# soedinglab/plass

Measured on AMD Instinct MI355X. Metric: read-overlaps/s per assembly iteration, higher is better.
Workload: dtype u8/u64 (integer hash, byte compare; f32 ratios)

## Files before the change

plass_amd/csrc/common.hpp:

```cpp
#pragma once
#include <hip/hip_runtime.h>
#include <cstdint>
#include <cstddef>
#include <cstdio>
#include <atomic>
#include <functional>
#include <memory>
#include <mutex>
#include <string>
#include <vector>
#include "../../include/plasship.h"

namespace plasship {

void setError(const std::string &msg);
hipError_t streamSync(hipStream_t st);
}
struct plasship_seqdb; struct plasship_ctx;
namespace plasship {
int ensureOffLen(plasship_ctx *ctx, const plasship_seqdb *db);
std::string hipErrStr(hipError_t e, const char *what, const char *file, int line);

#define PH_CHECK(call)                                                                   \
    do {                                                                                 \
        hipError_t e_ = (call);                                                          \
        if (e_ != hipSuccess) {                                                          \
            plasship::setError(plasship::hipErrStr(e_, #call, __FILE__, __LINE__));     \
            return PLASSHIP_ERR_DEVICE;                                                  \
        }                                                                                \
    } while (0)
#define PH_COPY_SYNC(st, dst, src, bytes, kind)                                          \
    do {                                                                                 \
        PH_CHECK(hipMemcpyAsync((dst), (src), (bytes), (kind), (st)));                   \
        PH_CHECK(plasship::streamSync(st));                                              \
    } while (0)

int tuneInt(const char *name, int dflt);
bool traceOn();
#define PH_TRACE(st, what)                                                                \
    do {                                                                                 \
        if (plasship::traceOn()) {                                                       \
            hipError_t e_ = plasship::streamSync(st);                                    \
            fprintf(stderr, "[plasship] %s: %s\n", (what), hipGetErrorString(e_));       \
        }                                                                                \
    } while (0)

hipError_t poolMalloc(void **p, size_t n, bool longLived = false);
void poolEnter(hipStream_t stream);
void watchEnter(const plasship_ctx *ctx);
void watchCollective(const char *what);
#define PH_ENTER(ctx)                                                                    \
    do {                                                                                 \
        PH_CHECK(hipSetDevice((ctx)->device));                                           \
        plasship::poolEnter((ctx)->stream);                                              \
        plasship::watchEnter(ctx);                                                       \
    } while (0)
void poolFree(void *p);
void poolTrim();

struct DevBuf {
    void *p = nullptr; size_t bytes = 0;
    DevBuf() {}
    DevBuf(const DevBuf &) = delete; DevBuf &operator=(const DevBuf &) = delete;
    ~DevBuf() { release(); }
    hipError_t alloc(size_t n, bool longLived = false) { release(); bytes = n; if (n == 0) { p = nullptr; return hipSuccess; } return poolMalloc(&p, n, longLived); }
    hipError_t allocLong(size_t n) { return alloc(n, true); }
    void release() { if (p) { poolFree(p); p = nullptr; } bytes = 0; }
    template <typename T> T *as() const { return reinterpret_cast<T *>(p); }
};

struct SeqView {
    const char *data;
    const uint64_t *off;
    const uint32_t *len;
    const uint64_t *offLen;
    uint32_t n;
    int nucl;
};

#ifdef __HIPCC__
__device__ __forceinline__ uint64_t seqOff(const SeqView &s, uint32_t id) { return s.offLen[id] >> 24; }
__device__ __forceinline__ uint32_t seqLen(const SeqView &s, uint32_t id) { return (uint32_t) s.offLen[id] & 0xFFFFFFu; }
#endif

struct __attribute__((aligned(8))) CandHit { uint32_t target; int32_t prefScore; uint32_t diag16; uint32_t query; };

struct AlnRec {
    uint32_t query, target;
    int32_t bitScore, rawScore;
    float seqId;
    int32_t qStart, qEnd, qLen, dbStart, dbEnd, dbLen, alnLen;
    int32_t reversed;
    int32_t accepted;
    int32_t fromText;
    int32_t btKind;
};
constexpr int32_t ALN_SELF_PENDING = 3;

}

struct plasship_ctx {
    int device = 0;
    hipStream_t stream = nullptr;
    hipEvent_t ev[16] = {};
    int numCU = 0;
    std::vector<uint32_t> ambKeys;
    std::vector<uint8_t> ambVals;
    plasship::DevBuf d_ambKeys, d_ambVals;
    plasship::DevBuf d_cmpCache;
    uint32_t ambSlots = 0;
    char *stage[2] = {nullptr, nullptr};
    hipEvent_t stageEv[2] = {nullptr, nullptr};
    size_t stageBytes = 0;
    void *pinnedTable = nullptr;
    bool hasComm = false;
    plasship_comm comm = {};
    int debugFailCollective = -1;
    struct KmCache {
        plasship::DevBuf lines; uint64_t n = 0, gen = 0; bool valid = false, seenEligible = false;
        int k = 0, alph = 0, kps = 0, ignoreMulti = 0, hashShift = 0;
    } kmCache;
    struct KmPosCache {
        plasship::DevBuf pos, slotOff, idHash; uint64_t n = 0, gen = 0; bool valid = false, seen = false, lng = false;
        int k = 0, kps = 0, ignoreMulti = 0, hashShift = 0; float scale = 0;
    } kmPosCache;
    uint64_t kmermatchCalls = 0;
    uint64_t cycKnownGen = 0, cycKnownMaxLen = 0;
};

namespace plasship {
uint64_t newDbGeneration();
struct SeqHeap { DevBuf buf; std::atomic<uint64_t> used{0}; };
}
struct plasship_seqdb {
    int dbtype = 0;
    uint64_t gen = plasship::newDbGeneration(), parentGen = 0, ancestorGen = 0;
    plasship::DevBuf d_changed;
    uint64_t originGen = 0;
    plasship::DevBuf d_origin;
    size_t n = 0;
    uint64_t dataBytes = 0, residues = 0;
    uint32_t maxEntryLen = 0;
    plasship::DevBuf d_data, d_off, d_len, d_key;
    std::shared_ptr<plasship::SeqHeap> heap;
    bool contiguous = true;
    uint64_t buildAppendedBytes = 0, buildCopiedBytes = 0;
    const char *borrowedData = nullptr;
    const char *dataPtr() const { return heap ? heap->buf.as<char>() : borrowedData ? borrowedData : d_data.as<char>(); }
    plasship::DevBuf d_fileRank;
    mutable plasship::DevBuf d_offLen;
    mutable std::mutex offLenMu; mutable hipEvent_t offLenEv = nullptr; mutable hipStream_t offLenStream = nullptr;
    ~plasship_seqdb() { if (offLenEv) (void) hipEventDestroy(offLenEv); }
    bool hostIndexValid = false;
    std::vector<uint32_t> h_key, h_elen;
    std::vector<uint64_t> h_off;
    plasship::SeqView view() const {
        plasship::SeqView v; v.data = dataPtr(); v.off = d_off.as<uint64_t>(); v.len = d_len.as<uint32_t>(); v.offLen = d_offLen.as<uint64_t>();
        v.n = (uint32_t) n; v.nucl = (dbtype == PLASSHIP_DBTYPE_NUCLEOTIDES); return v;
    }
};

struct plasship_cands {
    bool reverseCapable = false;
    size_t nQueries = 0;
    uint64_t nHits = 0;
    uint64_t nNonSelf = 0;
    plasship::DevBuf d_qoff;
    plasship::DevBuf d_hits;
};

struct plasship_alns {
    size_t nQueries = 0;
    uint64_t nLines = 0;
    uint64_t nSlots = 0;
    bool sparse = false;
    mutable bool selfPending = false;
    plasship_rescore_params rsPar = {};
    bool rsSameDB = false; int rsReverseCapable = 0;
    bool nucl = false;
    bool addBacktrace = false;
    uint64_t dbResidues = 0;
    int gappedOpen = 0, gappedExtend = 0;
    plasship::DevBuf d_qoff;
    plasship::DevBuf d_recs;
    const plasship_seqdb *qdb = nullptr, *tdb = nullptr;
};

namespace plasship {
inline const plasship_comm *commOf(const plasship_ctx *ctx) { return ctx->hasComm ? &ctx->comm : nullptr; }
inline uint64_t ownedBegin(uint64_t n, int r, int world) { return ((uint64_t) r * n + (uint64_t) world - 1) / (uint64_t) world; }
int commAllgatherHost(plasship_ctx *ctx, const void *send, void *recv, uint64_t bytesPerRank);
int commAllReduceSumU64(plasship_ctx *ctx, uint64_t *v, size_t n);
int commAllReduceMaxU64(plasship_ctx *ctx, uint64_t *v, size_t n);
int commAllReduceMinU64(plasship_ctx *ctx, uint64_t *v, size_t n);
int commAgreeOk(plasship_ctx *ctx, bool ok, const char *what);
int commFinish(plasship_ctx *ctx, int rc);
int commAlltoallvRecords(plasship_ctx *ctx, const void *dSend, const uint64_t *sendCount, size_t recordBytes, DevBuf &recv,
                         uint64_t *recvTotal, uint64_t slackRecords, uint64_t *allTotal = nullptr);
int commAllgathervBytes(plasship_ctx *ctx, const void *dSend, uint64_t sendBytes, DevBuf &recv, std::vector<uint64_t> &recvBytes);
int commAllgathervBytesKnown(plasship_ctx *ctx, const void *dSend, uint64_t sendBytes, DevBuf &recv, const std::vector<uint64_t> &recvBytes);
int packedCopyOf(plasship_ctx *ctx, const plasship_seqdb *db, std::unique_ptr<plasship_seqdb> &out);
int buildOutputDB(plasship_ctx *ctx, const plasship_seqdb *db, const uint32_t *dFlags, const uint32_t *dNewLen, const uint64_t *dNewStart,
                  const char *dArena, int keepTarget, void *dTmp, size_t tmpBytes, plasship_seqdb **out,
                  const void *dExtra = nullptr, void *hExtra = nullptr, size_t extraBytes = 0, hipEvent_t doneEvent = nullptr, bool noAppend = false);
int stagedUpload(plasship_ctx *ctx, void *dDst, uint64_t total, const std::function<void(char *, uint64_t, uint64_t)> &produce,
                 uint64_t chunk = 0, const std::function<int(uint64_t)> *enqueued = nullptr);
int stagedDownload(plasship_ctx *ctx, const void *dSrc, uint64_t total, const std::function<bool(const char *, uint64_t, uint64_t)> &consume);
void *ctxPinnedTable(plasship_ctx *ctx, size_t bytes);
int stagedCopyToDevice(plasship_ctx *ctx, void *dDst, const void *hSrc, uint64_t bytes);
int stagedCopyToHost(plasship_ctx *ctx, void *hDst, const void *dSrc, uint64_t bytes);
int deviceKeysDiffer(plasship_ctx *ctx, const uint32_t *a, const uint32_t *b, size_t n, bool *differ);
int denseAlnsCopy(plasship_ctx *ctx, const plasship_alns *a, DevBuf &qoffBuf, DevBuf &recsBuf, const uint64_t **qoff, const AlnRec **recs);
int finishSelfAlns(plasship_ctx *ctx, const plasship_alns *a, const uint32_t *dQueryList = nullptr, uint32_t nQueryList = 0);
}
```

plass_amd/csrc/core.hip:

```cpp
#include "common.hpp"
#include "host_util.hpp"
#include "device_utils.hpp"
#include <algorithm>
#include <atomic>
#include <condition_variable>
#include <thread>
#include <memory>
#include <chrono>
#include <cstdio>
#include <cstdlib>
#include <cstring>
#include <map>
#include <mutex>
#include <numeric>
#include <unordered_map>
#include <unistd.h>

namespace plasship {
namespace {
std::mutex g_poolMu;
constexpr size_t POOL_ALIGN = 256;
struct FreeRange { size_t size; hipStream_t stream; bool mixed; };
struct Slab { char *base; size_t size; size_t used; std::map<size_t, FreeRange> free; };
struct DevicePool { std::vector<Slab> slabs; size_t total = 0; };
std::map<int, DevicePool> g_pools;
struct PoolLive { int device; int slab; size_t off, size; hipStream_t stream; };
std::unordered_map<void *, PoolLive> g_poolLive;
thread_local hipStream_t tl_poolStream = nullptr;
int g_ctxCount = 0;
std::mutex g_reserveMu; std::condition_variable g_reserveCv; int g_reserving = 0;
thread_local bool tl_isReserver = false;
struct ReserveJoin { ~ReserveJoin() { std::unique_lock<std::mutex> lk(g_reserveMu); g_reserveCv.wait(lk, [] { return g_reserving == 0; }); } } g_reserveJoin;
size_t g_poolHits = 0, g_poolMisses = 0; double g_poolMissMs = 0, g_poolMissBytes = 0;

bool takeRange(DevicePool &dp, int dev, size_t n, void **p, hipStream_t *waitFor, bool *waitAll, bool longLived) {
    int bs = -1; size_t bo = 0, bsz = ~(size_t) 0; const char *bestEnd = nullptr;
    for (size_t i = 0; i < dp.slabs.size(); i++)
        for (auto &kv : dp.slabs[i].free) {
            if (kv.second.size < n) continue;
            if (longLived) {
                const char *end = dp.slabs[i].base + kv.first + kv.second.size;
                if (bs < 0 || dp.slabs[i].size > dp.slabs[bs].size || (dp.slabs[i].size == dp.slabs[bs].size && end > bestEnd)) { bs = (int) i; bo = kv.first; bsz = kv.second.size; bestEnd = end; }
            } else if (kv.second.size < bsz) { bs = (int) i; bo = kv.first; bsz = kv.second.size; }
        }
    if (bs < 0) return false;
    Slab &sl = dp.slabs[bs];
    const FreeRange fr = sl.free[bo];
    sl.free.erase(bo);
    size_t at = bo;
    if (longLived) { at = bo + fr.size - n; if (fr.size > n) sl.free[bo] = FreeRange{fr.size - n, fr.stream, fr.mixed}; }
    else if (fr.size > n) sl.free[bo + n] = FreeRange{fr.size - n, fr.stream, fr.mixed};
    sl.used += n;
    *p = sl.base + at;
    bo = at;
    g_poolLive[*p] = PoolLive{dev, bs, bo, n, tl_poolStream};
    *waitAll = fr.mixed; *waitFor = (!fr.mixed && fr.stream != tl_poolStream) ? fr.stream : nullptr;
    return true;
}
void trimLocked(int onlyDevice) {
    int cur = 0; (void) hipGetDevice(&cur);
    for (auto &dv : g_pools) {
        if (onlyDevice >= 0 && dv.first != onlyDevice) continue;
        bool any = false; for (auto &sl : dv.second.slabs) any |= (sl.used == 0 && sl.base != nullptr);
        if (!any) continue;
        (void) hipSetDevice(dv.first); (void) hipDeviceSynchronize();
        for (auto &sl : dv.second.slabs) if (sl.used == 0 && sl.base) { (void) hipFree(sl.base); dv.second.total -= sl.size; sl.base = nullptr; sl.size = 0; sl.free.clear(); }
    }
    (void) hipSetDevice(cur);
}
}
static int poisonByte() { static const int v = [] { const char *e = getenv("PLASSHIP_POOL_POISON"); return e ? atoi(e) : -1; }(); return v; }
static hipError_t poolMallocRaw(void **p, size_t n, bool longLived);
hipError_t poolMalloc(void **p, size_t n, bool longLived) {
    const hipError_t e = poolMallocRaw(p, n, longLived);
    if (e == hipSuccess && poisonByte() >= 0) { (void) hipDeviceSynchronize(); (void) hipMemset(*p, poisonByte(), n); (void) hipDeviceSynchronize(); }
    return e;
}
void poolEnter(hipStream_t stream) { tl_poolStream = stream; }
static void poolForgetStream(hipStream_t stream) {
    std::lock_guard<std::mutex> g(g_poolMu);
    for (auto &dv : g_pools) for (auto &sl : dv.second.slabs) for (auto &kv : sl.free) if (!kv.second.mixed && kv.second.stream == stream) kv.second.stream = nullptr;
    for (auto &kv : g_poolLive) if (kv.second.stream == stream) kv.second.stream = nullptr;
    if (tl_poolStream == stream) tl_poolStream = nullptr;
}
static double poolFraction() { static const double v = [] { const char *e = getenv("PLASSHIP_POOL_FRACTION"); const double x = e ? atof(e) : 0.0; return (x > 0.05 && x <= 0.98) ? x : 0.88; }(); return v; }
static hipError_t poolMallocRaw(void **p, size_t n, bool longLived) {
    n = std::max<size_t>((n + POOL_ALIGN - 1) / POOL_ALIGN * POOL_ALIGN, POOL_ALIGN);
    int dev = 0; (void) hipGetDevice(&dev);
    const size_t MB2 = (size_t) 2 << 20;
    for (int fails = 0;;) {
        hipStream_t waitFor = nullptr; bool waitAll = false, hit = false;
        size_t slabBytes = 0;
        {
            std::lock_guard<std::mutex> g(g_poolMu);
            DevicePool &dp = g_pools[dev];
            hit = takeRange(dp, dev, n, p, &waitFor, &waitAll, longLived);
            if (hit) g_poolHits++;
            else {
                size_t fr = 0, tt = 0; (void) hipMemGetInfo(&fr, &tt);
                const size_t keepFree = (size_t) 3 << 29;
                const size_t most = std::min<size_t>((size_t) ((double) fr * poolFraction()), fr > keepFree ? fr - keepFree : 0);
                bool haveBigSlab = false;
                for (const auto &sl : dp.slabs) if (sl.base && sl.size >= ((size_t) 16 << 30)) haveBigSlab = true;
                const bool bigJob = !haveBigSlab && (dp.total >= ((size_t) 8 << 30) || n >= ((size_t) 4 << 30));
                slabBytes = bigJob ? most : std::min<size_t>(std::max<size_t>(2 * n, (size_t) 1 << 30), most);
                if (slabBytes < n || fails) slabBytes = n;
                slabBytes = (slabBytes + MB2 - 1) / MB2 * MB2;
            }
        }
        if (hit) {
            if (waitAll) (void) hipDeviceSynchronize();
            else if (waitFor) (void) plasship::streamSync(waitFor);
            return hipSuccess;
        }
        if (!tl_isReserver) {
            std::unique_lock<std::mutex> lk(g_reserveMu);
            if (g_reserving) { g_reserveCv.wait(lk, [] { return g_reserving == 0; }); continue; }
        }
        const auto t0 = std::chrono::steady_clock::now();
        void *base = nullptr;
        const hipError_t e = hipMalloc(&base, slabBytes);
        const double ms = std::chrono::duration<double, std::milli>(std::chrono::steady_clock::now() - t0).count();
        std::lock_guard<std::mutex> g(g_poolMu);
        if (e != hipSuccess) {
            (void) hipGetLastError();
            if (++fails >= 3) return e;
            trimLocked(dev);
            continue;
        }
        DevicePool &dp = g_pools[dev];
        Slab sl; sl.base = static_cast<char *>(base); sl.size = slabBytes; sl.used = 0; sl.free[0] = FreeRange{slabBytes, nullptr, false};
        size_t idx = dp.slabs.size();
        for (size_t i = 0; i < dp.slabs.size(); i++) if (!dp.slabs[i].base) { idx = i; break; }
        if (idx == dp.slabs.size()) dp.slabs.push_back(std::move(sl)); else dp.slabs[idx] = std::move(sl);
        dp.total += slabBytes; g_poolMisses++; g_poolMissMs += ms; g_poolMissBytes += (double) slabBytes;
    }
}
void poolFree(void *p) {
    std::lock_guard<std::mutex> g(g_poolMu);
    auto it = g_poolLive.find(p);
    if (it == g_poolLive.end()) { (void) hipFree(p); return; }
    const PoolLive lv = it->second;
    g_poolLive.erase(it);
    Slab &sl = g_pools[lv.device].slabs[lv.slab];
    sl.used -= lv.size;
    size_t off = lv.off, size = lv.size; hipStream_t stream = lv.stream; bool mixed = (tl_poolStream != nullptr && tl_poolStream != lv.stream);
    auto nx = sl.free.lower_bound(off);
    if (nx != sl.free.end() && off + size == nx->first) {
        if (nx->second.mixed || nx->second.stream != stream) mixed = !(nx->second.stream == nullptr && !nx->second.mixed) || mixed;
        size += nx->second.size; nx = sl.free.erase(nx);
    }
    if (nx != sl.free.begin()) {
        auto pv = std::prev(nx);
        if (pv->first + pv->second.size == off) {
            if (pv->second.mixed || pv->second.stream != stream) mixed = !(pv->second.stream == nullptr && !pv->second.mixed) || mixed;
            off = pv->first; size += pv->second.size; sl.free.erase(pv);
        }
    }
    sl.free[off] = FreeRange{size, stream, mixed};
}
void poolTrim() {
    std::lock_guard<std::mutex> g(g_poolMu);
    trimLocked(-1);
}
static thread_local std::string g_err;
int tuneInt(const char *name, int dflt) {
    char key[96]; snprintf(key, sizeof(key), "PLASSHIP_TUNE_%s", name);
    const char *e = getenv(key); const int v = e ? atoi(e) : 0;
    return v > 0 ? v : dflt;
}
static const char *const TUNE_NAMES[] = {"AGGWAVE", "AGGWAVE_CAP", "ASMQ", "ASMQ_CAP", "ROWTIER", "KMCACHE", "FORCE_LONG", "CYC_PASSES", "CYCSKIP", "SHARD_EXTRACT",
                                         "FASTA_CHUNK_MB", "DBHEAP", "DBHEAP_GB", "LAZY_SELF", "FASTQ_CHUNK_KB"};
static void reportUnknownTunes() {
    static const char PREFIX[] = "PLASSHIP_TUNE_";
    for (char **e = environ; e && *e; e++) {
        if (strncmp(*e, PREFIX, sizeof(PREFIX) - 1) != 0) continue;
        const char *x = *e + sizeof(PREFIX) - 1, *eq = strchr(x, '=');
        const std::string name(x, eq ? (size_t) (eq - x) : strlen(x));
        bool known = false;
        for (const char *k : TUNE_NAMES) known = known || name == k;
        if (!known) fprintf(stderr, "[plasship] PLASSHIP_TUNE_%s is not a switch of this build (ignored)\n", name.c_str());
    }
}
bool traceOn() { static const bool v = getenv("PLASSHIP_TRACE") != nullptr; return v; }
void setError(const std::string &msg) { g_err = msg; }
static std::atomic<unsigned long long> g_hostSyncs(0);
thread_local int tl_watchRank = -1, tl_watchWorld = 1;
thread_local const char *tl_watchLast = "none yet";
thread_local unsigned long long tl_watchCount = 0;
thread_local std::string tl_watchMsg;
void watchEnter(const plasship_ctx *ctx) {
    if (ctx && ctx->hasComm && ctx->comm.world > 1) { tl_watchRank = ctx->comm.rank; tl_watchWorld = ctx->comm.world; }
    else { tl_watchRank = -1; tl_watchWorld = 1; }
    tl_watchMsg.clear();
}
void watchCollective(const char *what) { tl_watchLast = what; tl_watchCount++; }
static double commTimeoutSeconds() { static const double v = [] { const char *e = getenv("PLASSHIP_COMM_TIMEOUT_S"); return e ? atof(e) : 300.0; }(); return v; }
hipError_t streamSync(hipStream_t st) {
    g_hostSyncs++;
    const double limit = tl_watchWorld > 1 ? commTimeoutSeconds() : 0.0;
    if (limit <= 0.0) return hipStreamSynchronize(st);
    const auto t0 = std::chrono::steady_clock::now();
    for (unsigned spins = 0;; spins++) {
        const hipError_t e = hipStreamQuery(st);
        if (e != hipErrorNotReady) return e;
        if (spins < 512) continue;
        const double el = std::chrono::duration<double>(std::chrono::steady_clock::now() - t0).count();
        if (el > limit) {
            tl_watchMsg = "sharded run, rank " + std::to_string(tl_watchRank) + " of " + std::to_string(tl_watchWorld) + ": the stream did not drain within " + std::to_string((int) limit) +
                          " s (PLASSHIP_COMM_TIMEOUT_S); last collective enqueued: " + tl_watchLast + " (#" + std::to_string(tl_watchCount) + " on this thread) - a peer that left the call, "
                          "or a link that is down (NCCL_DEBUG=INFO shows RCCL's view)";
            fprintf(stderr, "[plasship] %s\n", tl_watchMsg.c_str());
            return hipErrorNotReady;
        }
        std::this_thread::sleep_for(std::chrono::microseconds(el < 0.01 ? 20 : 200));
    }
}
std::string hipErrStr(hipError_t e, const char *what, const char *file, int line) {
    const std::string std_ = std::string("HIP error ") + hipGetErrorString(e) + " in " + what + " at " + file + ":" + std::to_string(line);
    if (!tl_watchMsg.empty()) { const std::string m = tl_watchMsg + " [" + std_ + "]"; tl_watchMsg.clear(); return m; }
    return std_;
}
__global__ void keysDifferKernel(const uint32_t *__restrict__ a, const uint32_t *__restrict__ b, uint32_t n, uint32_t *__restrict__ flag) {
    for (uint32_t i = blockIdx.x * blockDim.x + threadIdx.x; i < n; i += gridDim.x * blockDim.x) if (a[i] != b[i]) *flag = 1u;
}
int deviceKeysDiffer(plasship_ctx *ctx, const uint32_t *a, const uint32_t *b, size_t n, bool *differ) {
    DevBuf dFlag; uint32_t d = 0;
    if (dFlag.alloc(4) != hipSuccess) { setError("out of device memory"); return PLASSHIP_ERR_DEVICE; }
    PH_CHECK(hipMemsetAsync(dFlag.p, 0, 4, ctx->stream));
    if (n) hipLaunchKernelGGL(keysDifferKernel, dim3(std::min<uint32_t>(((uint32_t) n + 255) / 256, 1024)), dim3(256), 0, ctx->stream, a, b, (uint32_t) n, dFlag.as<uint32_t>());
    PH_COPY_SYNC(ctx->stream, &d, dFlag.p, 4, hipMemcpyDeviceToHost);
    *differ = d != 0;
    return PLASSHIP_OK;
}
}
using namespace plasship;

extern "C" const char *plasship_last_error(void) { return g_err.c_str(); }
extern "C" const char *plasship_version(void) { return "plasship 0.1 (gfx950)"; }

extern "C" int plasship_ctx_create(int device_ordinal, plasship_ctx **out) {
    if (!out) { setError("plasship_ctx_create: out is NULL"); return PLASSHIP_ERR_ARG; }
    static std::once_flag tunesChecked;
    std::call_once(tunesChecked, reportUnknownTunes);
    int count = 0;
    hipError_t e = hipGetDeviceCount(&count);
    if (e != hipSuccess || count == 0) {
        setError("plasship_ctx_create: no HIP device available (this library has no CPU fallback)");
        return PLASSHIP_ERR_DEVICE;
    }
    if (device_ordinal < 0) {
        const char *lr = getenv("LOCAL_RANK");
        device_ordinal = lr ? atoi(lr) % count : 0;
    }
    if (device_ordinal >= count) { setError("plasship_ctx_create: device ordinal out of range"); return PLASSHIP_ERR_ARG; }
    PH_CHECK(hipSetDevice(device_ordinal));
    std::unique_ptr<plasship_ctx> holder(new plasship_ctx());
    plasship_ctx *c = holder.get();
    c->device = device_ordinal;
    hipDeviceProp_t prop;
    PH_CHECK(hipGetDeviceProperties(&prop, device_ordinal));
    c->numCU = prop.multiProcessorCount;
    PH_CHECK(hipStreamCreateWithFlags(&c->stream, hipStreamNonBlocking));
    poolEnter(c->stream);
    for (auto &ev : c->ev) PH_CHECK(hipEventCreate(&ev));
    { std::lock_guard<std::mutex> g(g_poolMu); g_ctxCount++; }
    *out = holder.release();
    return PLASSHIP_OK;
}

extern "C" int plasship_ctx_reserve_async(plasship_ctx *ctx) {
    if (!ctx) { setError("plasship_ctx_reserve_async: ctx is NULL"); return PLASSHIP_ERR_ARG; }
    {
        std::lock_guard<std::mutex> g(g_poolMu);
        for (const auto &sl : g_pools[ctx->device].slabs) if (sl.base && sl.size >= ((size_t) 16 << 30)) return PLASSHIP_OK;
    }
    { std::lock_guard<std::mutex> lk(g_reserveMu); if (g_reserving) return PLASSHIP_OK; g_reserving = 1; }
    const int dev = ctx->device;
    std::thread([dev] {
        (void) hipSetDevice(dev);
        tl_isReserver = true;
        void *p = nullptr;
        if (poolMalloc(&p, (size_t) 4 << 30) == hipSuccess) poolFree(p);
        { std::lock_guard<std::mutex> lk(g_reserveMu); g_reserving = 0; }
        g_reserveCv.notify_all();
    }).detach();
    return PLASSHIP_OK;
}

uint64_t plasship::newDbGeneration() { static std::atomic<uint64_t> g(0); return ++g; }

extern "C" void plasship_ctx_destroy(plasship_ctx *ctx) {
    if (!ctx) return;
    (void) hipSetDevice(ctx->device);
    (void) plasship::streamSync(ctx->stream);
    for (auto &ev : ctx->ev) if (ev) (void) hipEventDestroy(ev);
    for (int i = 0; i < 2; i++) { if (ctx->stage[i]) (void) hipHostFree(ctx->stage[i]); if (ctx->stageEv[i]) (void) hipEventDestroy(ctx->stageEv[i]); }
    if (ctx->pinnedTable) (void) hipHostFree(ctx->pinnedTable);
    { std::unique_lock<std::mutex> lk(g_reserveMu); g_reserveCv.wait(lk, [] { return g_reserving == 0; }); }
    ctx->kmCache.lines.release(); ctx->d_cmpCache.release(); ctx->d_ambKeys.release(); ctx->d_ambVals.release();
    if (ctx->stream) { poolForgetStream(ctx->stream); (void) hipStreamDestroy(ctx->stream); }
    bool last; { std::lock_guard<std::mutex> g(g_poolMu); last = (--g_ctxCount <= 0); }
    if (last) {
        if (getenv("PLASSHIP_POOL_STATS")) fprintf(stderr, "plasship pool: %zu hits, %zu misses (%.1f ms in hipMalloc, %.1f MB)\n", g_poolHits, g_poolMisses, g_poolMissMs, g_poolMissBytes / 1e6);
        poolTrim();
    }
    delete ctx;
}

extern "C" int plasship_ctx_sync(plasship_ctx *ctx) {
    if (!ctx) { setError("ctx is NULL"); return PLASSHIP_ERR_ARG; }
    PH_CHECK(plasship::streamSync(ctx->stream));
    return PLASSHIP_OK;
}
extern "C" unsigned long long plasship_host_syncs(void) { return plasship::g_hostSyncs.load(); }
extern "C" void *plasship_ctx_stream(plasship_ctx *ctx) { return ctx ? (void *) ctx->stream : nullptr; }

namespace plasship {
static int stageReady(plasship_ctx *ctx) {
    if (ctx->stageBytes) return PLASSHIP_OK;
    size_t want = 32u << 20;
    if (const char *e = getenv("PLASSHIP_STAGE_MB")) { const long v = atol(e); if (v >= 1 && v <= 4096) want = (size_t) v << 20; }
    for (int i = 0; i < 2; i++) {
        PH_CHECK(hipHostMalloc((void **) &ctx->stage[i], want, hipHostMallocDefault));
        PH_CHECK(hipEventCreateWithFlags(&ctx->stageEv[i], hipEventDisableTiming));
    }
    ctx->stageBytes = want;
    return PLASSHIP_OK;
}
void *ctxPinnedTable(plasship_ctx *ctx, size_t bytes) {
    if (bytes > (1u << 20)) return nullptr;
    if (!ctx->pinnedTable && hipHostMalloc(&ctx->pinnedTable, 1u << 20, hipHostMallocDefault) != hipSuccess) { ctx->pinnedTable = nullptr; (void) hipGetLastError(); }
    return ctx->pinnedTable;
}
int stagedUpload(plasship_ctx *ctx, void *dDst, uint64_t total, const std::function<void(char *, uint64_t, uint64_t)> &produce,
                 uint64_t chunk, const std::function<int(uint64_t)> *enqueued) {
    if (!total) return PLASSHIP_OK;
    int rc = stageReady(ctx); if (rc) return rc;
    const uint64_t CH = chunk ? std::min<uint64_t>(chunk, ctx->stageBytes) : ctx->stageBytes; int b = 0; bool used[2] = {false, false};
    for (uint64_t o = 0; o < total; o += CH, b ^= 1) {
        const uint64_t n = std::min<uint64_t>(CH, total - o);
        if (used[b]) PH_CHECK(hipEventSynchronize(ctx->stageEv[b]));
        produce(ctx->stage[b], o, n);
        PH_CHECK(hipMemcpyAsync((char *) dDst + o, ctx->stage[b], n, hipMemcpyHostToDevice, ctx->stream));
        PH_CHECK(hipEventRecord(ctx->stageEv[b], ctx->stream)); used[b] = true;
        if (enqueued) { rc = (*enqueued)(o + n); if (rc) { (void) plasship::streamSync(ctx->stream); return rc; } }
    }
    PH_CHECK(plasship::streamSync(ctx->stream));
    return PLASSHIP_OK;
}
int stagedDownload(plasship_ctx *ctx, const void *dSrc, uint64_t total, const std::function<bool(const char *, uint64_t, uint64_t)> &consume) {
    if (!total) return PLASSHIP_OK;
    int rc = stageReady(ctx); if (rc) return rc;
    const uint64_t CH = ctx->stageBytes;
    auto issue = [&](uint64_t o, int b) -> int {
        const uint64_t n = std::min<uint64_t>(CH, total - o);
        PH_CHECK(hipMemcpyAsync(ctx->stage[b], (const char *) dSrc + o, n, hipMemcpyDeviceToHost, ctx->stream));
        PH_CHECK(hipEventRecord(ctx->stageEv[b], ctx->stream));
        return PLASSHIP_OK;
    };
    rc = issue(0, 0); if (rc) return rc;
    int b = 0;
    for (uint64_t o = 0; o < total; o += CH, b ^= 1) {
        if (o + CH < total) { rc = issue(o + CH, b ^ 1); if (rc) return rc; }
        PH_CHECK(hipEventSynchronize(ctx->stageEv[b]));
        if (!consume(ctx->stage[b], o, std::min<uint64_t>(CH, total - o))) { (void) plasship::streamSync(ctx->stream); return PLASSHIP_ERR_IO; }
    }
    return PLASSHIP_OK;
}
static void parallelCopy(char *dst, const char *src, uint64_t n) {
    const size_t SL = 1u << 20;
    parallelRanges((size_t) ((n + SL - 1) / SL), [&](int, size_t b, size_t e) {
        const uint64_t o = (uint64_t) b * SL, end = std::min<uint64_t>(n, (uint64_t) e * SL);
        if (end > o) memcpy(dst + o, src + o, (size_t) (end - o));
    }, nullptr, 4);
}
int stagedCopyToDevice(plasship_ctx *ctx, void *dDst, const void *hSrc, uint64_t bytes) {
    return stagedUpload(ctx, dDst, bytes, [&](char *dst, uint64_t o, uint64_t n) { parallelCopy(dst, (const char *) hSrc + o, n); });
}
int stagedCopyToHost(plasship_ctx *ctx, void *hDst, const void *dSrc, uint64_t bytes) {
    return stagedDownload(ctx, dSrc, bytes, [&](const char *src, uint64_t o, uint64_t n) { parallelCopy((char *) hDst + o, src, n); return true; });
}
}
using namespace plasship;

namespace plasship {
__global__ __launch_bounds__(256) void validateBytesKernel(const uint4 *__restrict__ data, uint64_t nWords, const uint64_t *__restrict__ off, uint64_t n, unsigned long long *__restrict__ counts) {
    unsigned long long hi = 0, zero = 0, bad = 0;
    for (uint64_t i = (uint64_t) blockIdx.x * 256 + threadIdx.x; i < nWords; i += (uint64_t) gridDim.x * 256) {
        const uint4 w = data[i];
        const uint32_t v[4] = {w.x, w.y, w.z, w.w};
#pragma unroll
        for (int j = 0; j < 4; j++) {
            const uint32_t x = v[j];
            hi += (unsigned) __popc((((x & 0x7F7F7F7Fu) + 0x05050505u) | x) & 0x80808080u);
            zero += (unsigned) __popc(~(((x & 0x7F7F7F7Fu) + 0x7F7F7F7Fu) | x | 0x7F7F7F7Fu));
        }
    }
    const char *bytes = reinterpret_cast<const char *>(data);
    for (uint64_t i = (uint64_t) blockIdx.x * 256 + threadIdx.x; i < n; i += (uint64_t) gridDim.x * 256) bad += bytes[off[i + 1] - 1] != 0;
    hi = waveReduceSumU64(hi); zero = waveReduceSumU64(zero); bad = waveReduceSumU64(bad);
    if ((threadIdx.x & 63) == 0) { if (hi) atomicAdd(&counts[0], hi); if (zero) atomicAdd(&counts[1], zero); if (bad) atomicAdd(&counts[2], bad); }
}
}

extern "C" int plasship_seqdb_upload(plasship_ctx *ctx, const char *data, size_t data_bytes, const uint64_t *off,
                                     const uint32_t *elen, const uint32_t *key, size_t n, int dbtype,
                                     plasship_seqdb **out) {
    if (!ctx || !out || (n && (!data || !off || !elen || !key))) { setError("plasship_seqdb_upload: bad argument"); return PLASSHIP_ERR_ARG; }
    if (dbtype != PLASSHIP_DBTYPE_AMINO_ACIDS && dbtype != PLASSHIP_DBTYPE_NUCLEOTIDES) {
        setError("plasship_seqdb_upload: dbtype must be amino acids (0) or nucleotides (1)"); return PLASSHIP_ERR_UNSUPPORTED;
    }
    if (n >= 0xFFFFFFFFull) { setError("plasship_seqdb_upload: too many sequences"); return PLASSHIP_ERR_UNSUPPORTED; }
    PH_ENTER(ctx);
    std::vector<uint32_t> perm(n);
    std::atomic<bool> sortedA(true);
    parallelRanges(n, [&](int, size_t b, size_t e) {
        bool ok = true;
        for (size_t i = b; i < e; i++) { perm[i] = (uint32_t) i; if (i > 0 && key[i - 1] > key[i]) ok = false; }
        if (!ok) sortedA = false;
    });
    const bool sorted = sortedA;
    const double tu0 = ioNow();
    if (!sorted) std::stable_sort(perm.begin(), perm.end(), [&](uint32_t a, uint32_t b) { return key[a] < key[b]; });
    std::unique_ptr<plasship_seqdb> holder(new plasship_seqdb());
    plasship_seqdb *db = holder.get();
    db->dbtype = dbtype; db->n = n;
    db->h_key.resize(n); db->h_elen.resize(n); db->h_off.resize(n);
    std::vector<uint32_t> hlen(n);
    uint64_t total = 0; uint32_t maxE = 0;
    {
        const int maxT = hostThreads();
        std::vector<uint64_t> rangeSum((size_t) maxT + 1, 0), rangeBeg((size_t) maxT + 1, 0); std::vector<uint32_t> rangeMax((size_t) maxT + 1, 0);
        std::vector<std::pair<size_t, size_t>> ranges((size_t) maxT + 1, std::make_pair((size_t) 0, (size_t) 0));
        std::atomic<int> bad(0);
        const int used = parallelRanges(n, [&](int t, size_t b, size_t e) {
            uint64_t sum = 0; uint32_t mx = 0;
            for (size_t i = b; i < e; i++) {
                const uint32_t sI = perm[i];
                if (off[sI] + elen[sI] > data_bytes) { bad = 1; return; }
                if (elen[sI] < 2) { bad = 2; return; }
                sum += elen[sI]; mx = std::max(mx, elen[sI]);
            }
            rangeSum[(size_t) t] = sum; rangeMax[(size_t) t] = mx; ranges[(size_t) t] = std::make_pair(b, e);
        });
        if (bad == 1) { setError("plasship_seqdb_upload: entry beyond data"); return PLASSHIP_ERR_ARG; }
        if (bad == 2) { setError("plasship_seqdb_upload: sequence entry shorter than \"\\n\\0\""); return PLASSHIP_ERR_ARG; }
        std::vector<int> order((size_t) used); for (int t = 0; t < used; t++) order[(size_t) t] = t;
        std::sort(order.begin(), order.end(), [&](int x, int y) { return ranges[(size_t) x].first < ranges[(size_t) y].first; });
        for (int q = 0; q < used; q++) { const int t = order[(size_t) q]; rangeBeg[(size_t) t] = total; total += rangeSum[(size_t) t]; maxE = std::max(maxE, rangeMax[(size_t) t]); }
        std::vector<std::pair<size_t, size_t>> rs(ranges.begin(), ranges.begin() + used);
        parallelRanges((size_t) used, [&](int, size_t qb, size_t qe) {
            for (size_t q = qb; q < qe; q++) {
                uint64_t o = rangeBeg[q];
                for (size_t i = rs[q].first; i < rs[q].second; i++) {
                    const uint32_t sI = perm[i];
                    db->h_key[i] = key[sI]; db->h_elen[i] = elen[sI]; db->h_off[i] = o; hlen[i] = elen[sI] - 2;
                    o += elen[sI];
                }
            }
        }, nullptr, 1);
    }
    db->dataBytes = total; db->maxEntryLen = maxE; db->residues = total - 2 * (uint64_t) n; db->hostIndexValid = true;
    if (db->d_data.allocLong(total + 64) != hipSuccess || db->d_off.allocLong((n + 1) * 8) != hipSuccess ||
        db->d_len.allocLong((n + 1) * 4) != hipSuccess || db->d_key.allocLong((n + 1) * 4) != hipSuccess) {
        setError("plasship_seqdb_upload: out of device memory"); return PLASSHIP_ERR_DEVICE;
    }
    const double tu1 = ioNow();
    PH_CHECK(hipMemsetAsync((char *) db->d_data.p + total, 0, 64, ctx->stream));
    {
        const uint64_t *newOff = db->h_off.data();
        const int rc = stagedUpload(ctx, db->d_data.p, total, [&](char *dst, uint64_t o, uint64_t nb) {
            const size_t first = (size_t) (std::upper_bound(newOff, newOff + n, o) - newOff) - 1;
            const size_t last = (size_t) (std::upper_bound(newOff, newOff + n, o + nb - 1) - newOff);
            parallelRanges(last - first, [&](int, size_t b, size_t e) {
                for (size_t i = first + b; i < first + e; i++) {
                    const uint64_t eb = newOff[i], ee = eb + db->h_elen[i];
                    const uint64_t cb = std::max(eb, o), ce = std::min(ee, o + nb);
                    if (ce > cb) memcpy(dst + (cb - o), data + off[perm[i]] + (cb - eb), (size_t) (ce - cb));
                }
            }, nullptr, 1024);
        });
        if (rc) return rc;
    }
    const double tu2 = ioNow();
    {
        bool fileSorted = true;
        for (size_t i = 1; i < n && fileSorted; i++) fileSorted = off[perm[i - 1]] <= off[perm[i]];
        if (!fileSorted) {
            std::vector<uint32_t> byOff(n), rank(n);
            std::iota(byOff.begin(), byOff.end(), 0u);
            std::stable_sort(byOff.begin(), byOff.end(), [&](uint32_t x, uint32_t y) { return off[perm[x]] < off[perm[y]]; });
            for (size_t r = 0; r < n; r++) rank[byOff[r]] = (uint32_t) r;
            if (db->d_fileRank.allocLong(n * 4) != hipSuccess) { setError("plasship_seqdb_upload: out of device memory"); return PLASSHIP_ERR_DEVICE; }
            const int rc = stagedCopyToDevice(ctx, db->d_fileRank.p, rank.data(), n * 4); if (rc) return rc;
        }
    }
    std::vector<uint64_t> hoff(n + 1);
    for (size_t i = 0; i < n; i++) hoff[i] = db->h_off[i];
    hoff[n] = total;
    { int rc = stagedCopyToDevice(ctx, db->d_off.p, hoff.data(), (n + 1) * 8); if (rc) return rc; }
    if (n) {
        int rc = stagedCopyToDevice(ctx, db->d_len.p, hlen.data(), n * 4); if (rc) return rc;
        rc = stagedCopyToDevice(ctx, db->d_key.p, db->h_key.data(), n * 4); if (rc) return rc;
    }
    unsigned long long bc[3] = {0, 0, 0};
    if (n) {
        DevBuf dBC;
        if (dBC.alloc(24) != hipSuccess) { setError("plasship_seqdb_upload: out of device memory"); return PLASSHIP_ERR_DEVICE; }
        PH_CHECK(hipMemsetAsync(dBC.p, 0, 24, ctx->stream));
        const uint64_t nWords = (total + 15) / 16;
        hipLaunchKernelGGL(validateBytesKernel, dim3((unsigned) std::min<uint64_t>((nWords + 255) / 256, (uint64_t) ctx->numCU * 16)), dim3(256), 0, ctx->stream,
                           (const uint4 *) db->d_data.p, nWords, (const uint64_t *) db->d_off.as<uint64_t>(), (uint64_t) n, dBC.as<unsigned long long>());
        PH_CHECK(hipMemcpyAsync(bc, dBC.p, 24, hipMemcpyDeviceToHost, ctx->stream));
    }
    PH_CHECK(plasship::streamSync(ctx->stream));
    if (ioTimingOn()) fprintf(stderr, "[plasship io] seqdb_upload: %zu entries, %.2f GB: host index arrays + device allocation (waits for the arena) %.3f s, packed upload %.3f s, index upload + validation %.3f s\n",
                              n, (double) total / 1e9, tu1 - tu0, tu2 - tu1, ioNow() - tu2);
    const unsigned long long padZeros = (16 - total % 16) % 16;
    if (bc[0]) { setError("plasship_seqdb_upload: " + std::to_string(bc[0]) + " byte(s) above 'z' (122) in the sequence data: not a sequence DB the kernels' score tables can index"); return PLASSHIP_ERR_ARG; }
    if (bc[2] || bc[1] != (unsigned long long) n + padZeros) {
        setError("plasship_seqdb_upload: every entry must end in \"\\n\\0\" and hold no other NUL byte (" + std::to_string(bc[2]) + " entries without the final NUL, " +
                 std::to_string((long long) bc[1] - (long long) padZeros) + " NUL bytes in " + std::to_string(n) + " entries)"); return PLASSHIP_ERR_ARG;
    }
    *out = holder.release();
    return PLASSHIP_OK;
}

extern "C" int plasship_seqdb_read(plasship_ctx *ctx, const char *db_path, plasship_seqdb **out) {
    if (!ctx || !db_path || !out) { setError("plasship_seqdb_read: bad argument"); return PLASSHIP_ERR_ARG; }
    HostDB h; std::string err;
    const double t0 = ioNow();
    if (!readDBFiles(db_path, h, err)) { setError(err); return PLASSHIP_ERR_IO; }
    const double t1 = ioNow();
    const int rc = plasship_seqdb_upload(ctx, h.data.data(), h.data.size(), h.off.data(), h.elen.data(), h.key.data(), h.key.size(), h.dbtype, out);
    if (ioTimingOn()) fprintf(stderr, "[plasship io] seqdb_read %s: files %.3f s, index arrays + upload + validation %.3f s\n", db_path, t1 - t0, ioNow() - t1);
    return rc;
}

static int ensureHostIndex(plasship_ctx *ctx, plasship_seqdb *db) {
    if (db->hostIndexValid) return PLASSHIP_OK;
    size_t n = db->n;
    db->h_key.resize(n); db->h_off.resize(n + 1); db->h_elen.resize(n);
    std::vector<uint32_t> len(n);
    PH_CHECK(plasship::streamSync(ctx->stream));
    { int rc = stagedCopyToHost(ctx, db->h_off.data(), db->d_off.p, (n + 1) * 8); if (rc) return rc; }
    if (n) {
        int rc = stagedCopyToHost(ctx, db->h_key.data(), db->d_key.p, n * 4); if (rc) return rc;
        rc = stagedCopyToHost(ctx, len.data(), db->d_len.p, n * 4); if (rc) return rc;
    }
    parallelRanges(n, [&](int, size_t b, size_t e) { for (size_t i = b; i < e; i++) db->h_elen[i] = len[i] + 2; });
    db->h_off.resize(n);
    db->hostIndexValid = true;
    return PLASSHIP_OK;
}

extern "C" int plasship_seqdb_info(const plasship_seqdb *db, size_t *n, uint64_t *residues, uint32_t *max_entry_len,
                                   int *dbtype, uint64_t *data_bytes) {
    if (!db) { setError("plasship_seqdb_info: db is NULL"); return PLASSHIP_ERR_ARG; }
    if (n) *n = db->n;
    if (residues) *residues = db->residues;
    if (max_entry_len) *max_entry_len = db->maxEntryLen;
    if (dbtype) *dbtype = db->dbtype;
    if (data_bytes) *data_bytes = db->dataBytes;
    return PLASSHIP_OK;
}

extern "C" int plasship_seqdb_download(plasship_ctx *ctx, const plasship_seqdb *cdb, char *data, uint64_t *off,
                                       uint32_t *elen, uint32_t *key) {
    if (!ctx || !cdb) { setError("plasship_seqdb_download: bad argument"); return PLASSHIP_ERR_ARG; }
    PH_ENTER(ctx);
    std::unique_ptr<plasship_seqdb> packedTmp;
    if (!cdb->contiguous) { const int rcP = packedCopyOf(ctx, cdb, packedTmp); if (rcP) return rcP; cdb = packedTmp.get(); }
    plasship_seqdb *db = const_cast<plasship_seqdb *>(cdb);
    int rc = ensureHostIndex(ctx, db); if (rc) return rc;
    PH_CHECK(plasship::streamSync(ctx->stream));
    if (data && db->dataBytes) { rc = stagedCopyToHost(ctx, data, db->dataPtr(), db->dataBytes); if (rc) return rc; }
    if (off) memcpy(off, db->h_off.data(), db->n * 8);
    if (elen) memcpy(elen, db->h_elen.data(), db->n * 4);
    if (key) memcpy(key, db->h_key.data(), db->n * 4);
    return PLASSHIP_OK;
}

extern "C" int plasship_seqdb_write(plasship_ctx *ctx, const plasship_seqdb *cdb, const char *db_path) {
    if (!ctx || !cdb || !db_path) { setError("plasship_seqdb_write: bad argument"); return PLASSHIP_ERR_ARG; }
    PH_ENTER(ctx);
    std::unique_ptr<plasship_seqdb> packedTmp;
    if (!cdb->contiguous) { const int rcP = packedCopyOf(ctx, cdb, packedTmp); if (rcP) return rcP; cdb = packedTmp.get(); }
    plasship_seqdb *db = const_cast<plasship_seqdb *>(cdb);
    int rc = ensureHostIndex(ctx, db); if (rc) return rc;
    PH_CHECK(plasship::streamSync(ctx->stream));
    std::string err; DBFileWriter w;
    const double tw0 = ioNow();
    if (!w.open(db_path, db->dbtype, err)) { setError(err); return PLASSHIP_ERR_IO; }
    std::atomic<bool> packed(true);
    parallelRanges(db->n, [&](int, size_t b, size_t e) {
        for (size_t i = b; i < e; i++) if (db->h_off[i] + db->h_elen[i] != (i + 1 < db->n ? db->h_off[i + 1] : db->dataBytes)) { packed = false; return; }
    });
    if (packed) {
// ... 82 lines not shown
```

plass_amd/csrc/kmermatch.hip:

```cpp
#include "common.hpp"
#include "device_utils.hpp"
#include "host_util.hpp"
#include "linepart.hpp"
#include "xxh64_u64.hpp"
#include <algorithm>
#include <memory>
#include <type_traits>
#include <cstdlib>
#include <climits>
#include <cstring>

namespace plasship {

#include "kmermatch_extract.hpp"
#include "kmermatch_group.hpp"
#include "kmermatch_repsort.hpp"
}
using namespace plasship;

namespace {

struct Timer {
    plasship_ctx *ctx; int slot;
    void start(int s) { slot = s; (void) hipEventRecord(ctx->ev[s], ctx->stream); }
// ... 510 lines not shown
        const uint32_t m = (uint32_t) trec.size();
        bool mayHit = false;
        if (m) {
            std::vector<uint64_t> cum(VH_BINS + 1, 0);
            for (uint32_t b = 0; b < VH_BINS; b++) cum[b + 1] = cum[b] + hVHistG[b];
            for (uint32_t j = 0; j < m && !mayHit; j++) { const uint32_t b = valueBin<NUCL>(trec[j].kmer, valueShift); mayHit = Nm >= cum[b] && Nm < cum[b + 1]; }
        }
        if (m && mayHit) {
            PH_CHECK(hipMemcpyAsync(dTRec.p, trec.data(), (size_t) m * sizeof(R), hipMemcpyHostToDevice, st));
            hipLaunchKernelGGL((rankLinesKernel<NUCL, LONG>), dim3(gridFor(finalCap * RPL, 256, (unsigned) numCU * 8)), dim3(256), 0, st, (const void *) finalRecs, finalTags, finalCap, geo.nb2 ? (const uint64_t *) dTot2.as<uint64_t>() : (const uint64_t *) nullptr,
                               (const void *) dTRec.p, m, dDiff.as<unsigned long long>());
            std::vector<unsigned long long> diff((size_t) m + 1);
            PH_CHECK(hipMemcpyAsync(diff.data(), dDiff.p, ((size_t) m + 1) * 8, hipMemcpyDeviceToHost, st));
            PH_CHECK(plasship::streamSync(st));
            if (cm) {
                static_assert(sizeof(unsigned long long) == sizeof(uint64_t), "");
                rc = commAllReduceSumU64(ctx, reinterpret_cast<uint64_t *>(diff.data()), diff.size()); if (rc) return rc;
            }
            unsigned long long rank = 0, expect = Nm;
            for (uint32_t j = 0; j < m; j++) {
                rank += diff[j];
                if (rank == expect) { res.stalePos.push_back((int64_t) trec[j].pos); expect++; }
                else if (rank > expect) break;
            }
        }
        PH_TRACE(st, "kmermatch: stale-record check (line store)");
    }

    PH_CHECK(hipEventRecord(ctx->ev[12], st));
    if (exch) { dL2.release(); if (!geo.nb2) dRx.release(); }
    else (finalRecs == dA.p ? dA : dB).release();
    dTag1.release(); dList1.release(); dTag2.release(); dList2.release(); dRxList.release();
    std::vector<std::pair<uint64_t, uint64_t>> arenas(gGrid);
    for (uint32_t j = 0; j < gGrid; j++) arenas[j] = std::make_pair(hArena[j] / RPL, hOutCnt[j]);
    DevBuf dTriples, dRepStart; uint64_t nTriples = 0;
    auto arenasConsumed = [&]() { if (exch) { if (geo.nb2) dRx.release(); else dArena.release(); } else (arenaBuf == dA.p ? dA : dB).release(); };
    if (NUCL && cm) rc = repSortLines<NUCL, LONG, false, NUCL>(ctx, arenaBuf, arenas, NmLocal, N, 0u, N, 0, arenasConsumed, dTriples, nTriples, &dRepStart);
    else rc = repSortLines<NUCL, LONG, false>(ctx, arenaBuf, arenas, NmLocal, N, 0u, N, 0, arenasConsumed, dTriples, nTriples, cm ? &dRepStart : nullptr);
    if (rc) return rc;
    if (cm) {
        DevBuf dOB; std::vector<uint64_t> ob((size_t) W + 1), sendCount(W);
        if (dOB.alloc(((size_t) W + 1) * 8) != hipSuccess) { setError("kmermatch: out of device memory"); return PLASSHIP_ERR_DEVICE; }
        hipLaunchKernelGGL(ownerBoundsKernel, dim3(1), dim3(256), 0, st, (const uint64_t *) dRepStart.as<uint64_t>(), (uint64_t) N, W, dOB.as<uint64_t>());
        PH_COPY_SYNC(st, ob.data(), dOB.p, ((size_t) W + 1) * 8, hipMemcpyDeviceToHost);
        for (int r = 0; r < W; r++) sendCount[r] = ob[r + 1] - ob[r];
        DevBuf dRxT; uint64_t gotT = 0;
        constexpr size_t xBytes = NUCL ? sizeof(TripleX) : sizeof(Triple);
        rc = commAlltoallvRecords(ctx, dTriples.p, sendCount.data(), xBytes, dRxT, &gotT, RPL); if (rc) return rc;
        res.exchangedTripleBytes = (nTriples - sendCount[rk]) * xBytes;
        PH_TRACE(st, "kmermatch: exchange 2 (aggregated triples)");
        dTriples.release(); dRepStart.release();
        const uint32_t repBase = (uint32_t) ownedBegin(N, rk, W), ownedN = (uint32_t) (ownedBegin(N, rk + 1, W) - repBase);
        DevBuf dMerged; uint64_t nMerged = 0;
        rc = repSortLines<NUCL, LONG, true>(ctx, dRxT.p, {std::make_pair((uint64_t) 0, gotT)}, gotT, ownedN, repBase, N, HALO_SLACK, [&]() { dRxT.release(); }, dMerged, nMerged, nullptr);
        if (rc) return rc;
        moveBuf(dA, dMerged);
        nTriples = nMerged;
    } else moveBuf(dA, dTriples);
    PH_CHECK(hipEventRecord(ctx->ev[13], st));
    PH_TRACE(st, "kmermatch: rep sort (line store)");
    PH_CHECK(hipGetLastError());
    res.triples = dA.p; res.nTriples = nTriples;
    { float msS = 0, msS2 = 0; (void) hipEventElapsedTime(&msS, ctx->ev[8], ctx->ev[9]); if (res.nPart == 2) (void) hipEventElapsedTime(&msS2, ctx->ev[10], ctx->ev[11]); res.msPart = msS + msS2; }
    return PLASSHIP_OK;
}


template <bool NUCL, bool LONG>
static int reduceToCandidates(plasship_ctx *ctx, const plasship_seqdb *db, void *cur, uint64_t nTriples, const std::vector<int64_t> &stalePos, uint32_t staleT,
                              std::unique_ptr<plasship_cands> &holder, uint64_t &Nc, float &msReduce, bool lazyClock = false) {
    hipStream_t st = ctx->stream;
    const uint32_t N = (uint32_t) db->n;
    Timer tm{ctx, 0};
    const plasship_comm *cm = commOf(ctx);
    const int W = cm ? cm->world : 1, rk = cm ? cm->rank : 0;
    const uint64_t repBase = ownedBegin(N, rk, W), ownedN = ownedBegin(N, rk + 1, W) - repBase;
    if (!lazyClock) tm.start(0);
    DevBuf dTmpHits, dEmit, dEpos, dPerRep, dQoff;
    if (dTmpHits.alloc(std::max<uint64_t>(nTriples, 1) * sizeof(CandHit)) != hipSuccess || dEmit.alloc((nTriples / 64 + 2) * 4) != hipSuccess ||
        dEpos.alloc((nTriples / 64 + 3) * 8) != hipSuccess || dPerRep.alloc(((size_t) N + 1) * 4) != hipSuccess) { setError("kmermatch: out of device memory"); return PLASSHIP_ERR_DEVICE; }
    DevBuf dScanTmp2; const size_t scanTmp2Bytes = exclusiveScanTmpBytes(std::max<uint64_t>(nTriples, N) + 2);
    if (dScanTmp2.alloc(scanTmp2Bytes) != hipSuccess) { setError("kmermatch: out of device memory"); return PLASSHIP_ERR_DEVICE; }
    uint64_t nHalo = 0;
    if (cm) {
        Triple *dTr = reinterpret_cast<Triple *>(cur);
        std::vector<Triple> head; uint64_t headCnt = 0;
        if (nTriples) {
            uint64_t want = std::min<uint64_t>(nTriples, 1024);
            for (;;) {
                head.resize(want);
                PH_COPY_SYNC(st, head.data(), dTr, want * sizeof(Triple), hipMemcpyDeviceToHost);
                headCnt = 0; while (headCnt < want && head[headCnt].target == head[0].target) headCnt++;
                if (headCnt < want || want == nTriples) break;
                want = std::min<uint64_t>(nTriples, want * 2);
            }
            head.resize(headCnt);
        }
        Triple last; memset(&last, 0, sizeof(last));
        if (nTriples) PH_COPY_SYNC(st, &last, dTr + (nTriples - 1), sizeof(Triple), hipMemcpyDeviceToHost);
        uint64_t hdr[2] = {nTriples, headCnt}; std::vector<uint64_t> hdrs(2 * (size_t) W);
        int rc = commAllgatherHost(ctx, hdr, hdrs.data(), 16); if (rc) return rc;
        uint64_t maxHead = 0, sumHead = 0; for (int r = 0; r < W; r++) { maxHead = std::max(maxHead, hdrs[2 * (size_t) r + 1]); sumHead += hdrs[2 * (size_t) r + 1]; }
        if (sumHead + stalePos.size() > HALO_SLACK) { setError("kmermatch: a (rep, target) run continues over more than 65536 records of other ranks"); return PLASSHIP_ERR_UNSUPPORTED; }
        std::vector<Triple> heads;
        if (maxHead) {
            std::vector<Triple> mine(maxHead); memset(mine.data(), 0, maxHead * sizeof(Triple));
            std::copy(head.begin(), head.end(), mine.begin());
            heads.resize(maxHead * (size_t) W);
            rc = commAllgatherHost(ctx, mine.data(), heads.data(), maxHead * sizeof(Triple)); if (rc) return rc;
        }
        if (nTriples) {
            std::vector<Triple> halo; bool open = true;
            for (int r = rk + 1; r < W && open; r++) {
                const uint64_t nr = hdrs[2 * (size_t) r], hr = hdrs[2 * (size_t) r + 1];
                if (nr == 0) continue;
                const Triple *hp = heads.data() + maxHead * (size_t) r;
                if (hp[0].target != last.target) { open = false; break; }
                halo.insert(halo.end(), hp, hp + hr);
                if (hr < nr) open = false;
            }
            if (open && !stalePos.empty() && staleT == last.target) {
                for (int64_t sp : stalePos) {
                    Triple t; t.rep = 0xFFFFFFFFu; t.target = staleT; t.diag = LONG ? (int32_t) sp : (int32_t) (int16_t) sp; t.cnt = 1u | 0x80000000u;
                    halo.push_back(t);
                }
            }
            nHalo = halo.size();
            if (nHalo) PH_COPY_SYNC(st, dTr + nTriples, halo.data(), nHalo * sizeof(Triple), hipMemcpyHostToDevice);
        }
        PH_CHECK(hipMemsetAsync(dPerRep.p, 0, ((size_t) N + 1) * 4, st));
        if (ownedN) hipLaunchKernelGGL(fillU32Kernel, dim3(gridFor(ownedN, 256, 4096)), dim3(256), 0, st, dPerRep.as<uint32_t>() + repBase, 1u, ownedN);
    } else
    hipLaunchKernelGGL(fillU32Kernel, dim3(gridFor((uint64_t) N + 1, 256, 4096)), dim3(256), 0, st, dPerRep.as<uint32_t>(), 1u, (uint64_t) N);
    if (nTriples) hipLaunchKernelGGL((reduceRunsKernel<NUCL>), dim3(gridFor(nTriples, 256, 65535)), dim3(256), 0, st, (const Triple *) cur, nTriples, nTriples + nHalo, dTmpHits.as<CandHit>(), dEmit.as<uint32_t>(), dPerRep.as<uint32_t>());
    const uint64_t nWaves = (nTriples + 63) / 64;
    if (exclusiveScanU32(st, dEmit.as<uint32_t>(), dEpos.as<uint64_t>(), nWaves, dScanTmp2.p, scanTmp2Bytes)) { setError("kmermatch: scan failed"); return PLASSHIP_ERR_DEVICE; }
    holder.reset(new plasship_cands());
    plasship_cands *c = holder.get();
    c->reverseCapable = NUCL; c->nQueries = N;
    if (c->d_qoff.alloc(((size_t) N + 1) * 8) != hipSuccess) { setError("kmermatch: out of device memory"); return PLASSHIP_ERR_DEVICE; }
    if (exclusiveScanU32(st, dPerRep.as<uint32_t>(), c->d_qoff.as<uint64_t>(), N, dScanTmp2.p, scanTmp2Bytes)) { setError("kmermatch: scan failed"); return PLASSHIP_ERR_DEVICE; }
    Nc = 0;
    PH_CHECK(hipMemcpyAsync(&Nc, dEpos.as<uint64_t>() + nWaves, 8, hipMemcpyDeviceToHost, st));
    PH_CHECK(plasship::streamSync(st));
    const uint32_t qLo = cm ? (uint32_t) repBase : 0u, qHi = cm ? (uint32_t) (repBase + ownedN) : N;
    c->nHits = Nc + (qHi - qLo); c->nNonSelf = Nc;
    if (c->d_hits.alloc(std::max<uint64_t>(c->nHits, 1) * sizeof(CandHit)) != hipSuccess) { setError("kmermatch: out of device memory"); return PLASSHIP_ERR_DEVICE; }
    if (qHi > qLo) hipLaunchKernelGGL(placeSelfKernel, dim3(gridFor(qHi - qLo, 256, 4096)), dim3(256), 0, st, c->d_qoff.as<uint64_t>(), qLo, qHi, c->d_hits.as<CandHit>());
    if (nTriples) hipLaunchKernelGGL(placeHitsKernel, dim3(gridFor(nTriples, 256, 65535)), dim3(256), 0, st, dTmpHits.as<CandHit>(), dEpos.as<uint64_t>(), nTriples, qLo, c->d_hits.as<CandHit>());
    if (lazyClock) PH_CHECK(hipEventRecord(ctx->ev[14], st)); else msReduce = tm.stop(1);
    PH_TRACE(st, "kmermatch: reduce");
    PH_CHECK(plasship::streamSync(st));
    PH_CHECK(hipGetLastError());
    if (!stalePos.empty() && nTriples > 0 && !cm) {
        const Triple *dTr = reinterpret_cast<const Triple *>(cur);
        std::vector<Triple> tail; uint64_t want = std::min<uint64_t>(nTriples, 4096);
        for (;;) {
            tail.resize(want);
            PH_COPY_SYNC(st, tail.data(), dTr + (nTriples - want), want * sizeof(Triple), hipMemcpyDeviceToHost);
            if (tail.front().target != staleT || want == nTriples) break;
            want = std::min<uint64_t>(nTriples, want * 2);
        }
        if (tail.back().target == staleT) {
            size_t b0 = tail.size(); while (b0 > 0 && tail[b0 - 1].target == staleT) b0--;
            for (size_t h0 = b0; h0 < tail.size(); h0++) {
                if (!(h0 == b0 || tail[h0].rep != tail[h0 - 1].rep)) continue;
                int32_t diagonal = tail[h0].diag, prevDiagonal = tail[h0].diag;
                uint64_t maxDiagonal = 0, diagonalCnt = 0, topScore = 0;
                int bestRev = NUCL ? ((tail[h0].cnt & 0x80000000u) == 0) : 0;
                for (size_t j = h0; j < tail.size(); j++) {
                    const uint64_t cc = tail[j].cnt & 0x7FFFFFFFu;
                    if (prevDiagonal == tail[j].diag) diagonalCnt += cc; else diagonalCnt = cc;
                    if (diagonalCnt >= maxDiagonal) { diagonal = tail[j].diag; maxDiagonal = diagonalCnt; if (NUCL) bestRev = ((tail[j].cnt & 0x80000000u) == 0); }
                    prevDiagonal = tail[j].diag; topScore += cc;
                }
                for (int64_t sp : stalePos) {
                    const int32_t d = LONG ? (int32_t) sp : (int32_t) (int16_t) sp;
                    if (prevDiagonal == d) diagonalCnt++; else diagonalCnt = 1;
                    if (diagonalCnt >= maxDiagonal) { diagonal = d; maxDiagonal = diagonalCnt; if (NUCL) bestRev = 0; }
                    prevDiagonal = d; topScore++;
                }
                const uint32_t rep = tail[h0].rep;
                if (rep == staleT) continue;
                uint64_t qn = 0;
                PH_COPY_SYNC(st, &qn, c->d_qoff.as<uint64_t>() + rep + 1, 8, hipMemcpyDeviceToHost);
                CandHit hh;
                PH_COPY_SYNC(st, &hh, c->d_hits.as<CandHit>() + (qn - 1), sizeof(CandHit), hipMemcpyDeviceToHost);
                if (hh.target != staleT || hh.query != rep) { setError("kmermatch: internal error while patching the last run"); return PLASSHIP_ERR_DEVICE; }
                hh.prefScore = bestRev ? -(int) topScore : (int) topScore; hh.diag16 = (uint32_t) (uint16_t) diagonal;
                PH_COPY_SYNC(st, c->d_hits.as<CandHit>() + (qn - 1), &hh, sizeof(CandHit), hipMemcpyHostToDevice);
            }
        }
    }
    return PLASSHIP_OK;
}

template <bool NUCL, bool LONG>
int kmermatchImpl(plasship_ctx *ctx, const plasship_seqdb *db, const plasship_kmermatch_params *par, plasship_cands **out,
                  plasship_kmermatch_stats *stats, bool overflowCheckEarly) {
    typedef Rec<LONG> R;
    hipStream_t st = ctx->stream;
    const uint32_t N = (uint32_t) db->n;
    const int k = par->kmer_size;
    float msExtract = 0;
    const plasship_comm *cm = commOf(ctx);
    const int W = cm ? cm->world : 1, rk = cm ? cm->rank : 0;

    DevBuf dBound, dSlotOff, dScanTmp;
    const size_t scanTmpBytes = exclusiveScanTmpBytes((size_t) N + 2) + (1u << 20);
    if (dBound.alloc(((size_t) N + 1) * 4) != hipSuccess || dSlotOff.alloc(((size_t) N + 2) * 8) != hipSuccess || dScanTmp.alloc(scanTmpBytes) != hipSuccess) {
        setError("kmermatch: out of device memory"); return PLASSHIP_ERR_DEVICE;
    }
    PH_CHECK(hipEventRecord(ctx->ev[0], st));
    if (N) hipLaunchKernelGGL(boundsKernel, dim3(gridFor(N, 256, 4096)), dim3(256), 0, st, db->d_len.as<uint32_t>(), N, k, par->kmers_per_seq, par->kmers_per_seq_scale, dBound.as<uint32_t>());
    if (exclusiveScanU32(st, dBound.as<uint32_t>(), dSlotOff.as<uint64_t>(), N, dScanTmp.p, scanTmpBytes)) { setError("kmermatch: scan failed"); return PLASSHIP_ERR_DEVICE; }
    uint64_t total = 0;
    uint32_t sLo = 0, sHi = N; uint64_t slotBias = 0, totalAll = 0;
    const bool filtered = cm && shardOwnerFiltered(W);
    if (cm && !filtered) {
        DevBuf dSplit; std::vector<uint64_t> hSplit(2 * (size_t) W + 2);
        if (dSplit.alloc(hSplit.size() * 8) != hipSuccess) { setError("kmermatch: out of device memory"); return PLASSHIP_ERR_DEVICE; }
        hipLaunchKernelGGL(splitIdsKernel, dim3(1), dim3(256), 0, st, dSlotOff.as<uint64_t>(), N, W, dSplit.as<uint64_t>());
        PH_COPY_SYNC(st, hSplit.data(), dSplit.p, hSplit.size() * 8, hipMemcpyDeviceToHost);
        sLo = (uint32_t) hSplit[rk]; sHi = (uint32_t) hSplit[rk + 1]; slotBias = hSplit[W + 1 + rk];
        total = hSplit[W + 1 + rk + 1] - slotBias;
        totalAll = hSplit[2 * (size_t) W + 1];
    } else {
    PH_CHECK(hipMemcpyAsync(&total, dSlotOff.as<uint64_t>() + N, 8, hipMemcpyDeviceToHost, st));
    PH_CHECK(plasship::streamSync(st));
    totalAll = total;
    }
    const uint32_t nMine = sHi - sLo;

    DevBuf dA, dB;
    if (cm && W > 1024) { setError("kmermatch: more than 1024 ranks"); return PLASSHIP_ERR_UNSUPPORTED; }
    const LineGeo geo = lineGeometry(total, LONG, ctx->numCU, cm ? totalAll : 0, W);
    const uint64_t recCap = std::max<uint64_t>(total, (uint64_t) RPL * ((cm && !filtered) ? geo.cap1 : std::max(geo.cap1, geo.cap2)));
    if (dA.alloc(std::max<uint64_t>(recCap, 1) * sizeof(R)) != hipSuccess || dB.alloc(std::max<uint64_t>(recCap, 1) * sizeof(R)) != hipSuccess) {
        setError("kmermatch: out of device memory for the k-mer record arrays (" + std::to_string(2 * recCap * sizeof(R)) + " bytes)"); return PLASSHIP_ERR_DEVICE;
    }

    DevBuf dMap, dOvIds, dOvCnt;
    if (dMap.alloc(256) != hipSuccess || dOvIds.alloc(((size_t) N + 1) * 4) != hipSuccess || dOvCnt.alloc(4) != hipSuccess) { setError("kmermatch: out of device memory"); return PLASSHIP_ERR_DEVICE; }
    const unsigned char *map = aa2numTable(NUCL, par->alphabet_size);
    PH_CHECK(hipMemcpyAsync(dMap.p, map, 256, hipMemcpyHostToDevice, st));
    PH_CHECK(hipMemsetAsync(dOvCnt.p, 0, 4, st));
    ExtractArgs ea; memset(&ea, 0, sizeof(ea));
    ea.s = db->view(); ea.slotOff = dSlotOff.as<uint64_t>(); ea.arr = dA.p; ea.map = dMap.as<unsigned char>();
    const int alph = NUCL ? 5 : par->alphabet_size;
    { uint64_t p = 1; for (int i = 0; i < 24; i++) { ea.powers[i] = p; p *= (uint64_t) (alph - 1); } }
    ea.k = k; ea.xCode = map[(int) 'X']; ea.kps = par->kmers_per_seq; ea.ignoreMulti = par->ignore_multi_kmer; ea.scale = par->kmers_per_seq_scale;
    ea.seed = (uint64_t) par->hash_shift; ea.overflowIds = dOvIds.as<uint32_t>(); ea.overflowCount = dOvCnt.as<uint32_t>();
    ea.idLo = sLo; ea.idHi = sHi; ea.slotBias = slotBias;
    constexpr int CAP = 128, CAP2 = NUCL ? 1024 : 128;
    DevBuf dWaveList, dWaveCount, dLongList, dLongCount, dKStats;
    constexpr uint32_t TIER0_WINDOWS = 256;
    if (dWaveList.alloc(((size_t) N + 1) * 4) != hipSuccess || dWaveCount.alloc(4) != hipSuccess || dLongList.alloc(((size_t) N + 1) * 4) != hipSuccess || dLongCount.alloc(4) != hipSuccess ||
        dKStats.alloc(64) != hipSuccess) { setError("kmermatch: out of device memory"); return PLASSHIP_ERR_DEVICE; }
    PH_CHECK(hipMemsetAsync(dWaveCount.p, 0, 4, st));
    PH_CHECK(hipMemsetAsync(dLongCount.p, 0, 4, st));
    PH_CHECK(hipMemsetAsync(dKStats.p, 0, 64, st));
    ea.kstats = dKStats.as<unsigned long long>();
    plasship_ctx::KmCache &kc = ctx->kmCache;
    const bool fastIndex = !NUCL && k <= 14 && ea.powers[1] <= 16;
    const bool cacheEligible = !NUCL && !LONG && (!cm || filtered) && fastIndex && k <= 16 && par->kmers_per_seq >= 1 && par->kmers_per_seq <= (int) KMC_POS + 1 && par->kmers_per_seq_scale == 0.0f &&
                               tuneInt("KMCACHE", 1) == 1;
    const bool cacheReuse = cacheEligible && kc.valid && kc.n == N && kc.gen == db->parentGen && db->d_changed.p && kc.k == k && kc.alph == par->alphabet_size &&
                            kc.kps == par->kmers_per_seq && kc.ignoreMulti == par->ignore_multi_kmer && kc.hashShift == par->hash_shift && !overflowCheckEarly;
    kc.valid = false;
    DevBuf dCachedList, dCachedCount;
    unsigned long long cacheLinesPtr = 0;
    const bool cacheWanted = cacheEligible && N && (cacheReuse || db->parentGen != 0 || db->ancestorGen != 0 || kc.seenEligible);
    if (cacheEligible) kc.seenEligible = true;
    if (cacheWanted) {
        if (kc.lines.bytes < (size_t) N * KMC_LINE) { kc.lines.release(); if (kc.lines.allocLong((size_t) N * KMC_LINE) != hipSuccess) { setError("kmermatch: out of device memory for the selected-window cache"); return PLASSHIP_ERR_DEVICE; } }
        cacheLinesPtr = (unsigned long long) (uintptr_t) kc.lines.p;
        if (cacheReuse) {
            if (dCachedList.alloc(((size_t) N + 1) * 4) != hipSuccess || dCachedCount.alloc(4) != hipSuccess) { setError("kmermatch: out of device memory"); return PLASSHIP_ERR_DEVICE; }
            PH_CHECK(hipMemsetAsync(dCachedCount.p, 0, 4, st));
        }
    } else kc.lines.release();
    typedef typename std::conditional<LONG, uint32_t, unsigned short>::type PosT;
    plasship_ctx::KmPosCache &pc = ctx->kmPosCache;
    const bool posEligible = NUCL && !cm && N && tuneInt("KMCACHE", 1) == 1;
    bool posReuse = posEligible && pc.valid && pc.gen != 0 && db->originGen == pc.gen && db->d_origin.p && pc.lng == LONG && pc.k == k && pc.kps == par->kmers_per_seq &&
                          pc.scale == par->kmers_per_seq_scale && pc.ignoreMulti == par->ignore_multi_kmer && pc.hashShift == par->hash_shift;
    bool posWanted = posEligible && (posReuse || db->parentGen != 0 || db->ancestorGen != 0 || db->originGen != 0 || pc.seen || ctx->kmermatchCalls > 0);
    if (posEligible) pc.seen = true;
    ctx->kmermatchCalls++;
    DevBuf dPosNew, dIdHashNew;
    unsigned long long cachePtrs[3] = {cacheLinesPtr, 0, 0};
    if (posWanted && (dPosNew.allocLong((size_t) (total + 1) * sizeof(PosT)) != hipSuccess || dIdHashNew.allocLong(((size_t) N + 1) * 8) != hipSuccess)) {
        dPosNew.release(); dIdHashNew.release(); posWanted = posReuse = false;
    }
    if (posWanted) {
        cachePtrs[1] = (unsigned long long) (uintptr_t) dPosNew.p; cachePtrs[2] = (unsigned long long) (uintptr_t) dIdHashNew.p;
        if (posReuse) {
            if (dCachedList.alloc(((size_t) N + 1) * 4) != hipSuccess || dCachedCount.alloc(4) != hipSuccess) { setError("kmermatch: out of device memory"); return PLASSHIP_ERR_DEVICE; }
            PH_CHECK(hipMemsetAsync(dCachedCount.p, 0, 4, st));
        }
    }
    PH_CHECK(hipMemcpyAsync(dKStats.as<unsigned long long>() + 4, cachePtrs, 24, hipMemcpyHostToDevice, st));
    PH_CHECK(hipEventRecord(ctx->ev[2], st));
    if (!NUCL && k <= 16 && nMine) {
        ShortArgs sa; memset(&sa, 0, sizeof(sa));
        sa.s = ea.s; sa.slotOff = ea.slotOff; sa.arr = ea.arr; sa.map = ea.map; sa.k = k; sa.xCode = ea.xCode; sa.kps = ea.kps; sa.ignoreMulti = ea.ignoreMulti;
        sa.scale = ea.scale; sa.seed = ea.seed; sa.base = (uint64_t) (alph - 1); sa.top = ea.powers[k - 1];
        { uint64_t b = sa.base; int tz = 0; while ((b & 1) == 0) { b >>= 1; tz++; } uint64_t inv = b; for (int i = 0; i < 6; i++) inv *= 2 - b * inv; sa.tz = tz; sa.inv = inv; }
        sa.waveList = dWaveList.as<uint32_t>(); sa.waveCount = dWaveCount.as<uint32_t>(); sa.kstats = dKStats.as<unsigned long long>();
        sa.longList = dLongList.as<uint32_t>(); sa.longCount = dLongCount.as<uint32_t>(); sa.longWindows = TIER0_WINDOWS;
        sa.hugeList = dOvIds.as<uint32_t>(); sa.hugeCount = dOvCnt.as<uint32_t>(); sa.hugeWindows = 64 * 16;
        sa.idLo = sLo; sa.idHi = sHi; sa.slotBias = slotBias;
        if (cacheReuse) { sa.changed = db->d_changed.as<unsigned char>(); sa.cachedList = dCachedList.as<uint32_t>(); sa.cachedCount = dCachedCount.as<uint32_t>(); }
        constexpr int KF = 14, HF = KF / 2;
        bool fast = k == KF;
        uint64_t pwH = 1; for (int i = 0; i < HF; i++) pwH *= sa.base;
        if (pwH * 2 >= (1ull << 32)) fast = false;
        sa.topLo = (uint32_t) (pwH / sa.base); sa.topHi = (uint32_t) ea.powers[KF - HF - 1]; sa.baseH = (uint32_t) pwH;
        const dim3 shortGrid(std::min<uint32_t>((nMine + 63) / 64, (uint32_t) ctx->numCU * (nMine > 20000000u ? 288u : 18u)));
        const bool allWork = (int64_t) db->maxEntryLen - 2 - k + 1 <= (int64_t) par->kmers_per_seq - 1;
        const size_t padLds = (size_t) (allWork ? 16 : 8) << 10;
        const bool staged = !LONG && allWork;
        if (fast && sa.base < (1u << 8) && sa.topLo < (1u << 24) && sa.topHi < (1u << 24) && staged) {
            if constexpr (!LONG) hipLaunchKernelGGL((extractShortFastKernel<LONG, KF, true, true>), shortGrid, dim3(64), 0, st, sa);
        }
        else if (fast && sa.base < (1u << 8) && sa.topLo < (1u << 24) && sa.topHi < (1u << 24)) hipLaunchKernelGGL((extractShortFastKernel<LONG, KF, true>), shortGrid, dim3(64), padLds, st, sa);
        else if (fast) hipLaunchKernelGGL((extractShortFastKernel<LONG, KF, false>), shortGrid, dim3(64), 0, st, sa);
        else hipLaunchKernelGGL((extractShortKernel<LONG>), shortGrid, dim3(64), 0, st, sa);
        ea.waveList = dWaveList.as<uint32_t>(); ea.waveCount = dWaveCount.as<uint32_t>();
        if (cacheReuse) {
            CachedArgs ca; memset(&ca, 0, sizeof(ca));
            ca.s = ea.s; ca.slotOff = ea.slotOff; ca.arr = ea.arr; ca.map = ea.map; ca.lines = kc.lines.as<unsigned char>();
            ca.list = dCachedList.as<uint32_t>(); ca.count = dCachedCount.as<uint32_t>(); ca.k = k; ca.xCode = ea.xCode;
            ca.base = (uint32_t) ea.powers[1]; ca.base7 = (uint32_t) ea.powers[7]; ca.slotBias = slotBias; ca.seed = ea.seed; ca.kstats = dKStats.as<unsigned long long>();
            hipLaunchKernelGGL(extractCachedKernel, dim3(std::min<uint32_t>(nMine, (uint32_t) ctx->numCU * 32u)), dim3(64), 0, st, ca);
        }
    }
    else if (nMine) {
        hipLaunchKernelGGL(classifyWindowsKernel, dim3(std::min<uint32_t>((nMine + 2047) / 2048, (uint32_t) ctx->numCU * 8)), dim3(256), 0, st, (const uint32_t *) db->d_len.as<uint32_t>(), sLo, sHi, (uint32_t) k,
                           TIER0_WINDOWS, 64u * 16u, dWaveList.as<uint32_t>(), dWaveCount.as<uint32_t>(), dLongList.as<uint32_t>(), dLongCount.as<uint32_t>(), dOvIds.as<uint32_t>(), dOvCnt.as<uint32_t>(),
                           posReuse ? (const uint32_t *) db->d_origin.as<uint32_t>() : (const uint32_t *) nullptr, dCachedList.as<uint32_t>(), dCachedCount.as<uint32_t>());
        ea.waveList = dWaveList.as<uint32_t>(); ea.waveCount = dWaveCount.as<uint32_t>();
        if constexpr (NUCL) {
            if (posReuse) {
                CachedPosArgs<LONG> ca; memset(&ca, 0, sizeof(ca));
                ca.s = ea.s; ca.slotOff = ea.slotOff; ca.arr = ea.arr; ca.map = ea.map; ca.posOld = pc.pos.p; ca.slotOffOld = pc.slotOff.as<uint64_t>();
                ca.idHashOld = pc.idHash.as<unsigned long long>(); ca.origin = db->d_origin.as<uint32_t>(); ca.posNew = dPosNew.p; ca.idHashNew = dIdHashNew.as<unsigned long long>();
                ca.list = dCachedList.as<uint32_t>(); ca.count = dCachedCount.as<uint32_t>(); ca.k = k; ca.seed = ea.seed; ca.kstats = dKStats.as<unsigned long long>();
                hipLaunchKernelGGL((extractCachedPosKernel<LONG>), dim3(std::min<uint32_t>(nMine, (uint32_t) ctx->numCU * 32u)), dim3(64), 0, st, ca);
            }
        }
    }
    PH_CHECK(hipEventRecord(ctx->ev[3], st));
    PH_CHECK(hipEventRecord(ctx->ev[4], st));
    const int waveBlocksPerCU = nMine > 5000000u ? 192 : 32;
    DevBuf dOv2Ids, dOv2Cnt;
    DevBuf *lastIds = &dOvIds, *lastCnt = &dOvCnt;
    if (nMine) {
        if (dOv2Ids.alloc(((size_t) N + 1) * 4) != hipSuccess || dOv2Cnt.alloc(4) != hipSuccess) { setError("kmermatch: out of device memory"); return PLASSHIP_ERR_DEVICE; }
        PH_CHECK(hipMemsetAsync(dOv2Cnt.p, 0, 4, st));
        const uint32_t wide = std::min<uint32_t>(nMine, (uint32_t) ctx->numCU * (uint32_t) waveBlocksPerCU);
        ExtractArgs e0 = ea;
        DevBuf dRowLists, dRowCounts, dRowFall, dRowFallCnt;
        const bool rowTier = !NUCL && !LONG && fastIndex && k <= 14 && par->kmers_per_seq >= 1 && par->kmers_per_seq <= (int) KMC_POS + 1 &&
                             par->kmers_per_seq_scale == 0.0f && (tuneInt("ROWTIER", nMine > 4000000u ? 1 : 2) & 1) == 1;
        if (rowTier) {
            const uint32_t rs = N + 1;
            if (dRowLists.alloc((size_t) 4 * rs * 4) != hipSuccess || dRowCounts.alloc(16) != hipSuccess || dRowFall.alloc((size_t) rs * 4) != hipSuccess || dRowFallCnt.alloc(4) != hipSuccess) {
                setError("kmermatch: out of device memory"); return PLASSHIP_ERR_DEVICE;
            }
            PH_CHECK(hipMemsetAsync(dRowCounts.p, 0, 16, st));
            PH_CHECK(hipMemsetAsync(dRowFallCnt.p, 0, 4, st));
            hipLaunchKernelGGL(binWaveListKernel, dim3(std::min<uint32_t>((nMine + 2047) / 2048, (uint32_t) ctx->numCU * 8)), dim3(256), 0, st, (const uint32_t *) dWaveList.as<uint32_t>(), (const uint32_t *) dWaveCount.as<uint32_t>(),
                               (const uint32_t *) db->d_len.as<uint32_t>(), (uint32_t) k, 96u, 128u, 192u, dRowLists.as<uint32_t>(), rs, dRowCounts.as<uint32_t>());
            RowArgs ra; memset(&ra, 0, sizeof(ra));
            ra.s = ea.s; ra.slotOff = ea.slotOff; ra.arr = ea.arr; ra.map = ea.map; ra.fallList = dRowFall.as<uint32_t>(); ra.fallCount = dRowFallCnt.as<uint32_t>();
            ra.k = k; ra.xCode = ea.xCode; ra.kps = ea.kps; ra.ignoreMulti = ea.ignoreMulti; ra.seed = ea.seed; ra.base = (uint32_t) ea.powers[1]; ra.base7 = (uint32_t) ea.powers[7];
            ra.slotBias = slotBias; ra.kstats = dKStats.as<unsigned long long>();
            const dim3 rowGrid(std::min<uint32_t>((nMine + 3) / 4, (uint32_t) ctx->numCU * 32u));
            for (int b = 0; b < 4; b++) {
                ra.list = dRowLists.as<uint32_t>() + (size_t) b * rs; ra.count = dRowCounts.as<uint32_t>() + b;
                if (b == 0) hipLaunchKernelGGL((extractRowKernel<6>), rowGrid, dim3(64), 0, st, ra);
                else if (b == 1) hipLaunchKernelGGL((extractRowKernel<8>), rowGrid, dim3(64), 0, st, ra);
                else if (b == 2) hipLaunchKernelGGL((extractRowKernel<12>), rowGrid, dim3(64), 0, st, ra);
                else hipLaunchKernelGGL((extractRowKernel<16>), rowGrid, dim3(64), 0, st, ra);
            }
            e0.waveList = dRowFall.as<uint32_t>(); e0.waveCount = dRowFallCnt.as<uint32_t>();
        }
        hipLaunchKernelGGL((extractKernel<NUCL, LONG, CAP, false, 4, 256>), dim3(wide), dim3(64), 0, st, e0);
        ExtractArgs e1 = ea; e1.waveList = dLongList.as<uint32_t>(); e1.waveCount = dLongCount.as<uint32_t>();
        hipLaunchKernelGGL((extractKernel<NUCL, LONG, CAP, false, 16, 992>), dim3(wide), dim3(64), 0, st, e1);
        ExtractArgs e2 = ea; e2.waveList = dOvIds.as<uint32_t>(); e2.waveCount = dOvCnt.as<uint32_t>();
        e2.overflowIds = dOv2Ids.as<uint32_t>(); e2.overflowCount = dOv2Cnt.as<uint32_t>();
        constexpr int CAP48 = NUCL ? 512 : 128;
        if constexpr (NUCL) hipLaunchKernelGGL((extractKernel<NUCL, LONG, CAP48, false, 48, 992, 2>), dim3(std::min<uint32_t>(nMine, (uint32_t) ctx->numCU * 8u)), dim3(64), 0, st, e2);
        else hipLaunchKernelGGL((extractKernel<NUCL, LONG, CAP2, false, 48, 992>), dim3(std::min<uint32_t>(nMine, (uint32_t) ctx->numCU * 16u)), dim3(64), 0, st, e2);
        PH_CHECK(hipMemsetAsync(dOvCnt.p, 0, 4, st));
        ExtractArgs e3 = ea; e3.waveList = dOv2Ids.as<uint32_t>(); e3.waveCount = dOv2Cnt.as<uint32_t>();
        e3.overflowIds = dOvIds.as<uint32_t>(); e3.overflowCount = dOvCnt.as<uint32_t>();
        hipLaunchKernelGGL((extractKernel<NUCL, LONG, CAP2, false, 0, 8160>), dim3(std::min<uint32_t>(nMine, (uint32_t) ctx->numCU * (NUCL ? 2u : 5u))), dim3(64), 0, st, e3);
    }
    DevBuf &dLastIds = *lastIds, &dLastCnt = *lastCnt;
    PH_CHECK(hipEventRecord(ctx->ev[5], st));
    uint32_t nOv = 0;
    const bool overflowPossible = overflowCheckEarly || cm != nullptr || NUCL || db->maxEntryLen > 8160u || par->kmers_per_seq > 120 || par->kmers_per_seq_scale != 0.0f;
    if (nMine && overflowPossible) {
        PH_CHECK(hipMemcpyAsync(&nOv, dLastCnt.p, 4, hipMemcpyDeviceToHost, st));
        PH_CHECK(plasship::streamSync(st));
    } else if (nMine) hipLaunchKernelGGL((fillOverflowSlotsKernel<LONG>), dim3(64), dim3(64), 0, st, (const uint32_t *) dLastIds.as<uint32_t>(), (const uint32_t *) dLastCnt.as<uint32_t>(),
                                         (const uint64_t *) dSlotOff.as<uint64_t>(), slotBias, dA.p);
    PH_CHECK(hipGetLastError());
    if (nOv) {
        std::vector<uint32_t> ids(nOv), lens(nOv);
        DevBuf dLens, dSOff, dSCap, dScratch;
        if (dLens.alloc((size_t) nOv * 4) != hipSuccess) { setError("kmermatch: out of device memory"); return PLASSHIP_ERR_DEVICE; }
        hipLaunchKernelGGL(gatherU32Kernel, dim3(gridFor(nOv, 256, 1024)), dim3(256), 0, st, db->d_len.as<uint32_t>(), dLastIds.as<uint32_t>(), nOv, dLens.as<uint32_t>());
        PH_CHECK(hipMemcpyAsync(lens.data(), dLens.p, (size_t) nOv * 4, hipMemcpyDeviceToHost, st));
        PH_CHECK(plasship::streamSync(st));
        std::vector<uint64_t> soff(nOv); std::vector<uint32_t> scap(nOv); uint64_t tot = 0;
        for (uint32_t i = 0; i < nOv; i++) { uint32_t c = 64; while (c < lens[i] + 1) c <<= 1; scap[i] = c; soff[i] = tot; tot += c; }
        if (dSOff.alloc((size_t) nOv * 8) != hipSuccess || dSCap.alloc((size_t) nOv * 4) != hipSuccess || dScratch.alloc(tot * sizeof(Cand)) != hipSuccess) {
            setError("kmermatch: out of device memory for the long-sequence scratch"); return PLASSHIP_ERR_DEVICE;
        }
        PH_CHECK(hipMemcpyAsync(dSOff.p, soff.data(), (size_t) nOv * 8, hipMemcpyHostToDevice, st));
        PH_CHECK(hipMemcpyAsync(dSCap.p, scap.data(), (size_t) nOv * 4, hipMemcpyHostToDevice, st));
        ExtractArgs fa = ea; fa.idList = dLastIds.as<uint32_t>(); fa.nIds = nOv; fa.scratch = dScratch.as<Cand>(); fa.scratchOff = dSOff.as<uint64_t>(); fa.scratchCap = dSCap.as<uint32_t>();
        hipLaunchKernelGGL((extractKernel<NUCL, LONG, 1, true>), dim3(std::min<uint32_t>(nOv, (uint32_t) ctx->numCU * 8)), dim3(64), 0, st, fa);
        PH_CHECK(plasship::streamSync(st));
        PH_CHECK(hipGetLastError());
    }
    PH_TRACE(st, "kmermatch: extraction");
    traceBadIds<LONG>(ctx, "kmermatch: extracted slots", dA.p, total, N);

    {
        int keyBitsL = 0;
        if (NUCL) keyBitsL = 2 * k; else { long double v = 1; for (int i = 0; i < k; i++) v *= (long double) (alph - 1); while (keyBitsL < 63 && (long double) (1ULL << keyBitsL) < v) keyBitsL++; }
        LinesOut lo;
        int rcL = kmermatchLines<NUCL, LONG>(ctx, db, par, geo, total, dA, dB, dSlotOff, dKStats, ea, keyBitsL, lo, (nMine && !overflowPossible) ? dLastCnt.as<uint32_t>() : nullptr, filtered);
        if (rcL) return rcL;
        std::unique_ptr<plasship_cands> holderL; uint64_t NcL = 0; float msReduceL = 0;
        rcL = reduceToCandidates<NUCL, LONG>(ctx, db, lo.triples, lo.nTriples, lo.stalePos, lo.staleT, holderL, NcL, msReduceL, true);
        if (rcL) return rcL;
        {
            auto ms = [&](int a, int b) { float v = 0; (void) hipEventElapsedTime(&v, ctx->ev[a], ctx->ev[b]); return v; };
            msExtract = ms(0, 1); lo.msSort1 = ms(1, 6); lo.msGroup = ms(6, 7); lo.msSort2 = ms(12, 13); msReduceL = ms(13, 14);
        }
        if (stats) {
            stats->n_kmer_records = lo.Nk; stats->n_grouped = lo.Nm; stats->n_candidates = NcL; stats->record_bytes = LONG ? 20 : 16;
            float ms = 0, ms2 = 0; (void) hipEventElapsedTime(&ms, ctx->ev[2], ctx->ev[3]); (void) hipEventElapsedTime(&ms2, ctx->ev[4], ctx->ev[5]);
            stats->ms_extract_short_kernel = ms; stats->ms_extract_wave_kernel = ms2; stats->ms_extract_kernel = ms + ms2;
            stats->ms_part_scatter = lo.msPart; stats->n_part_scatter = lo.nPart;
            unsigned long long ks[4] = {0, 0, 0, 0}; uint32_t nCachedSeqs = 0;
            if (cacheReuse || posReuse) PH_CHECK(hipMemcpyAsync(&nCachedSeqs, dCachedCount.p, 4, hipMemcpyDeviceToHost, st));
            PH_COPY_SYNC(st, ks, dKStats.p, 32, hipMemcpyDeviceToHost);
            stats->n_cached_sequences = nCachedSeqs; stats->reserved0 = 0;
            stats->short_residues = ks[0]; stats->short_records = ks[1]; stats->wave_residues = ks[2]; stats->wave_records = ks[3];
            stats->residues = db->residues;
            stats->ms_extract = msExtract; stats->ms_sort1 = lo.msSort1; stats->ms_group = lo.msGroup; stats->ms_sort2 = lo.msSort2; stats->ms_reduce = msReduceL;
            stats->n_scratch_sequences = nOv; stats->n_restarts = overflowCheckEarly ? 1u : 0u;
        }
        if (cacheWanted) {
            kc.valid = true; kc.n = N; kc.gen = db->gen; kc.k = k; kc.alph = par->alphabet_size; kc.kps = par->kmers_per_seq; kc.ignoreMulti = par->ignore_multi_kmer; kc.hashShift = par->hash_shift;
        }
        if (posWanted) {
            if (pc.slotOff.allocLong(((size_t) N + 2) * 8) != hipSuccess) { pc.valid = false; setError("kmermatch: out of device memory for the position cache"); return PLASSHIP_ERR_DEVICE; }
            PH_CHECK(hipMemcpyAsync(pc.slotOff.p, dSlotOff.p, ((size_t) N + 1) * 8, hipMemcpyDeviceToDevice, st));
            PH_CHECK(plasship::streamSync(st));
            std::swap(pc.pos.p, dPosNew.p); std::swap(pc.pos.bytes, dPosNew.bytes); std::swap(pc.idHash.p, dIdHashNew.p); std::swap(pc.idHash.bytes, dIdHashNew.bytes);
            pc.valid = true; pc.n = N; pc.gen = db->gen; pc.lng = LONG; pc.k = k; pc.kps = par->kmers_per_seq; pc.scale = par->kmers_per_seq_scale;
            pc.ignoreMulti = par->ignore_multi_kmer; pc.hashShift = par->hash_shift;
        }
        *out = holderL.release();
        return PLASSHIP_OK;
    }
}
}

extern "C" int plasship_kmermatch(plasship_ctx *ctx, const plasship_seqdb *db, const plasship_kmermatch_params *par,
                                  plasship_cands **out, plasship_kmermatch_stats *stats) {
    if (!ctx || !db || !par || !out) { setError("plasship_kmermatch: bad argument"); return PLASSHIP_ERR_ARG; }
    const bool nucl = db->dbtype == PLASSHIP_DBTYPE_NUCLEOTIDES;
    if (par->kmer_size < 2 || par->kmer_size > (nucl ? 31 : 23)) { setError("plasship_kmermatch: unsupported k"); return PLASSHIP_ERR_UNSUPPORTED; }
    if (!nucl && par->alphabet_size != 13 && par->alphabet_size != 21) { setError("plasship_kmermatch: --alph-size must be 13 or 21"); return PLASSHIP_ERR_UNSUPPORTED; }
    if (db->maxEntryLen >= (1u << 20)) { setError("plasship_kmermatch: sequences of 2^20 residues or more are not supported"); return PLASSHIP_ERR_UNSUPPORTED; }
    PH_ENTER(ctx);
    const bool lng = !(db->maxEntryLen < (uint32_t) SHRT_MAX) || (nucl && par->kmer_size > 23) || tuneInt("FORCE_LONG", 0) == 1;
    int rc = KM_RETRY_EARLY_OVERFLOW_CHECK;
    for (int attempt = 0; attempt < 2 && rc == KM_RETRY_EARLY_OVERFLOW_CHECK; attempt++) {
        const bool early = attempt > 0;
        if (nucl) rc = lng ? kmermatchImpl<true, true>(ctx, db, par, out, stats, early) : kmermatchImpl<true, false>(ctx, db, par, out, stats, early);
        else rc = lng ? kmermatchImpl<false, true>(ctx, db, par, out, stats, early) : kmermatchImpl<false, false>(ctx, db, par, out, stats, early);
    }
    return commFinish(ctx, rc);
}
```

plass_amd/csrc/kmermatch_extract.hpp:

```cpp
#pragma once

__device__ __forceinline__ uint64_t revComplementDev(uint64_t kmer, int k) {
    uint64_t x = kmer ^ 0xAAAAAAAAAAAAAAAAULL;
    x = ((x >> 2) & 0x3333333333333333ULL) | ((x & 0x3333333333333333ULL) << 2);
    x = ((x >> 4) & 0x0F0F0F0F0F0F0F0FULL) | ((x & 0x0F0F0F0F0F0F0F0FULL) << 4);
    x = __builtin_bswap64(x);
    return x >> (64 - 2 * k);
}

__global__ void boundsKernel(const uint32_t *__restrict__ len, uint32_t n, int k, int kps, float scale, uint32_t *__restrict__ bound) {
    for (uint32_t i = blockIdx.x * blockDim.x + threadIdx.x; i < n; i += gridDim.x * blockDim.x) {
        const int L = (int) len[i];
        const int adj = max(1, L - k + 2);
        bound[i] = (uint32_t) min(adj, (int) ((float) (size_t) kps + (scale * (float) L)));
    }
}

struct Cand { uint64_t kmer; uint32_t pos; uint32_t score; };
constexpr uint32_t KMC_LINE = 128, KMC_POS = 59, KMC_FLAGS = 63, KMC_CLEAN = 1;

#define FALLBACK_NOSTATS(a) ((a).kstats == nullptr)
struct ExtractArgs {
    SeqView s;
    const uint64_t *slotOff;
// ... 287 lines not shown
                        else if (windowKmer(p, kmer, pos)) sc[j] = xxh64Score16(NUCL ? (kmer & ~BIT63) : kmer, a.seed);
                    }
                    n += (uint32_t) __popcll(__ballot(sc[j] != 0xFFFFFFFFu));
                }
            }
            considered = min(consideredRaw, (size_t) n);
            if (!allCand && considered > 0) {
                uint32_t t = 0;
                if (phaseSplit & 2) t = 1;
                else
#pragma unroll 1
                for (int bit = 15; bit >= 0; bit--) {
                    const uint32_t tr = t | (1u << bit);
                    uint32_t below = 0;
#pragma unroll
                    for (int j = 0; j < REGS; j++) if ((uint32_t) j * 64u < nWinU) below += (uint32_t) __popcll(__ballot(sc[j] < tr));
                    if ((size_t) below < considered) t = tr;
                }
                sStar = t;
                uint32_t upTo = 0;
#pragma unroll
                for (int j = 0; j < REGS; j++) if ((uint32_t) j * 64u < nWinU) upTo += (uint32_t) __popcll(__ballot(sc[j] <= t));
                tooMuch = (int) upTo - (int) considered;
            }
            if (allCand || considered > 0) {
#pragma unroll
                for (int j = 0; j < REGS; j++) {
                    if ((uint32_t) j * 64u < nWinU) {
                        const bool push = sc[j] != 0xFFFFFFFFu && (allCand || sc[j] <= sStar);
                        const unsigned long long mask = __ballot(push);
                        const uint32_t rank = (uint32_t) __popcll(mask & ((1ULL << lane) - 1ULL));
                        const uint32_t cnt = (uint32_t) __popcll(mask);
                        if (C + cnt > cap) overflow = true;
                        else if (push) sPick[C + rank] = (sc[j] << 16) | ((uint32_t) j * 64u + (uint32_t) lane);
                        C += cnt;
                    }
                }
            }
            __syncthreads();
            if (!overflow) {
                for (uint32_t i = lane; i < C; i += 64) {
                    const uint32_t pk = sPick[i];
                    Cand cd; uint32_t pos = 0; cd.kmer = pk;
                    if (!(phaseSplit & 4)) (void) windowKmer(pk & 0xFFFFu, cd.kmer, pos);
                    cd.pos = pos; cd.score = pk >> 16; cand[i] = cd;
                }
            }
            __syncthreads();
        } else {
        const int nPass = allCand ? 1 : 3;
        const bool resident = !FALLBACK && L <= RES_L;
        const bool useCache = resident && !allCand;
        if (resident) {
            for (uint32_t i = lane; i < L + 31; i += 64) {
                const char ch = (i < 64) ? cb0 : ((i < 128) ? cb1 : ((i < 192) ? cb2 : ((i < 256) ? cb3 : ((i < L) ? base[i] : (char) 0))));
                sCodeAll[i] = (i < L) ? sMap[(unsigned char) ch] : (unsigned char) a.xCode;
            }
            __syncthreads();
        }
        for (int pass = 0; pass < nPass; pass++) {
            if (pass < 2 && !allCand) { for (int i = lane; i < 256; i += 64) sHist[i] = 0; }
            __syncthreads();
            for (uint32_t t0 = 0; t0 < L; t0 += 64) {
                const uint32_t p = t0 + lane;
                bool valid; uint64_t kmer = 0; uint32_t pos = p, score = 0;
                const bool cached = useCache && pass > 0;
                if (!cached) {
                    unsigned char c;
                    if (resident) c = (p < L) ? sCodeAll[p] : (unsigned char) a.xCode;
                    else {
                        c = (p < L) ? sMap[(unsigned char) base[p]] : (unsigned char) a.xCode;
                        sCode[lane] = c;
                        if (lane < k - 1) { const uint32_t p2 = t0 + 64 + lane; sCode[64 + lane] = (p2 < L) ? sMap[(unsigned char) base[p2]] : (unsigned char) a.xCode; }
                    }
                    if (pass == 0) {
                        const uint32_t m = min(64u, L - t0);
                        const uint64_t pw = __shfl(pow31, (int) (m - 1 - min((uint32_t) lane, m - 1)), 64);
                        uint64_t term = ((uint32_t) lane < m) ? (uint64_t) c * pw : 0ull;
                        term = waveReduceSumU64(term);
                        const uint64_t pm = __shfl(pow31, (int) (m - 1), 64) * 31ull;
                        seqHash = seqHash * pm + term;
                    }
                    if (!resident) __syncthreads();
                    valid = (p < nWin);
                    if (valid) {
                        if (!NUCL && fastIdx) { pos = p; valid = kmerIndexFast(resident ? &sCodeAll[p] : &sCode[lane], k, (unsigned) a.xCode, (uint32_t) a.powers[1], (uint32_t) a.powers[7], kmer); }
                        else if (NUCL && a.xCode == 4) valid = kmerNuclCanonical(resident ? &sCodeAll[p] : &sCode[lane], k, L, p, kmer, pos);
                        else if (resident) valid = kmerFromCodes<NUCL>([&](int i) { return sCodeAll[p + i]; }, k, (unsigned char) a.xCode, a.powers, L, p, kmer, pos);
                        else valid = kmerFromCodes<NUCL>([&](int i) { return sCode[lane + i]; }, k, (unsigned char) a.xCode, a.powers, L, p, kmer, pos);
                    }
                    if (valid) score = xxh64Score16(NUCL ? (kmer & ~BIT63) : kmer, a.seed);
                    if (useCache) {
                        if (p < RES_L) sScore[p] = (unsigned short) score;
                        const unsigned long long vm = __ballot(valid);
                        if (lane == 0) sValid[t0 >> 6] = vm;
                    }
                } else {
                    valid = ((sValid[t0 >> 6] >> lane) & 1ULL) != 0;
                    score = valid ? (uint32_t) sScore[p] : 0u;
                    if (pass == 2 && valid && score <= sStar)
                    {
                        if (!NUCL && fastIdx) { pos = p; (void) kmerIndexFast(&sCodeAll[p], k, (unsigned) a.xCode, (uint32_t) a.powers[1], (uint32_t) a.powers[7], kmer); }
                        else if (NUCL && a.xCode == 4) (void) kmerNuclCanonical(&sCodeAll[p], k, L, p, kmer, pos);
                        else (void) kmerFromCodes<NUCL>([&](int i) { return sCodeAll[p + i]; }, k, (unsigned char) a.xCode, a.powers, L, p, kmer, pos);
                    }
                }
                bool push = false;
                if (allCand) push = valid;
                else if (pass == 0) { if (valid) atomicAdd(&sHist[score >> 8], 1u); }
                else if (pass == 1) { if (valid && (score >> 8) == b1) atomicAdd(&sHist[score & 255], 1u); }
                else push = valid && score <= sStar;
                if (pass == 0) n += (uint32_t) __popcll(__ballot(valid));
                if (allCand || pass == 2) {
                    const unsigned long long mask = __ballot(push);
                    const uint32_t rank = (uint32_t) __popcll(mask & ((1ULL << lane) - 1ULL));
                    const uint32_t cnt = (uint32_t) __popcll(mask);
                    if (C + cnt > cap) overflow = true;
                    else if (push) { Cand cd; cd.kmer = kmer; cd.pos = pos; cd.score = score; cand[C + rank] = cd; }
                    C += cnt;
                }
                __syncthreads();
                if (overflow) break;
            }
            if (overflow) break;
            if (!allCand && pass < 2) {
                __syncthreads();
                if (pass == 0) considered = min(consideredRaw, (size_t) n);
                const uint32_t target = (pass == 0) ? (uint32_t) considered : (uint32_t) considered - cumBefore1;
                const uint32_t h0 = sHist[lane * 4], h1 = sHist[lane * 4 + 1], h2 = sHist[lane * 4 + 2], h3 = sHist[lane * 4 + 3];
                const uint32_t mine = h0 + h1 + h2 + h3;
                const uint32_t incl = waveInclusiveScan(mine);
                const unsigned long long reach = __ballot(incl >= target && target > 0);
                uint32_t bin = 255, before = 0, upto = 0;
                if (reach) {
                    const int fl = __ffsll((long long) reach) - 1;
                    const uint32_t exB = __shfl(incl - mine, fl, 64);
                    const uint32_t q0 = __shfl(h0, fl, 64), q1 = __shfl(h1, fl, 64), q2 = __shfl(h2, fl, 64), q3 = __shfl(h3, fl, 64);
                    uint32_t run = exB; bin = (uint32_t) fl * 4;
                    if (run + q0 >= target) { before = run; upto = run + q0; }
                    else if (run + q0 + q1 >= target) { bin += 1; before = run + q0; upto = before + q1; }
                    else if (run + q0 + q1 + q2 >= target) { bin += 2; before = run + q0 + q1; upto = before + q2; }
                    else { bin += 3; before = run + q0 + q1 + q2; upto = before + q3; }
                }
                if (pass == 0) { b1 = bin; cumBefore1 = before; }
                else { sStar = (b1 << 8) | bin; tooMuch = (int) (cumBefore1 + upto) - (int) considered; }
                if (pass == 0 && (considered == 0)) break;
            }
        }
        }
        if (overflow) {
            if (!FALLBACK && lane == 0) { const uint32_t o = atomicAdd(a.overflowCount, 1u); a.overflowIds[o] = id; }
            __syncthreads();
            continue;
        }
        if (allCand) {
            considered = min(consideredRaw, (size_t) n);
            uint32_t mx = 0;
            for (uint32_t i = lane; i < C; i += 64) mx = max(mx, cand[i].score);
            sStar = (uint32_t) waveReduceMax((int) mx); tooMuch = 0;
        }
        bool needOrder = (tooMuch != 0);
        if (!needOrder && a.ignoreMulti && C > 1) {
            if (FALLBACK) needOrder = true;
            else {
                for (uint32_t i = lane; i < 2 * CAP; i += 64) sSet[i] = ~0ULL;
                __syncthreads();
                bool dup = false;
                for (uint32_t i = lane; i < C; i += 64) {
                    const unsigned long long K = NUCL ? (cand[i].kmer | BIT63) : cand[i].kmer;
                    uint32_t slot = (uint32_t) ((K * 0x9E3779B97F4A7C15ULL) >> 40) & (2 * CAP - 1);
                    for (;;) {
                        const unsigned long long prev = atomicCAS(&sSet[slot], ~0ULL, K);
                        if (prev == ~0ULL) break;
                        if (prev == K) { dup = true; break; }
                        slot = (slot + 1) & (2 * CAP - 1);
                    }
                }
                needOrder = __ballot(dup) != 0ULL;
                __syncthreads();
            }
        }
        if (!needOrder) {
            for (uint32_t i = lane; i < C; i += 64) {
                const Cand cd = cand[i];
                R r; r.kmer = cd.kmer; r.id = id; r.len = (decltype(r.len)) L; r.pos = (decltype(r.pos)) cd.pos;
                if constexpr (LONG) r.pad = 0;
                arr[slot + 1 + i] = r;
            }
            if (lane == 0) {
                R r; r.kmer = xxh64U64(seqHash, a.seed); r.id = id; r.len = (decltype(r.len)) L; r.pos = 0;
                if constexpr (LONG) r.pad = 0;
                arr[slot] = r;
            }
            for (uint32_t i = 1 + C + lane; i < bound; i += 64) { R r; memset(&r, 0xFF, sizeof(R)); arr[slot + i] = r; }
            if constexpr (NUCL) {
                if (!FALLBACK_NOSTATS(a)) {
                    PosT *pa = reinterpret_cast<PosT *>(a.kstats[5]);
                    if (pa) {
                        for (uint32_t i = lane; i < C; i += 64) { const Cand cd = cand[i]; pa[slot + 1 + i] = (PosT) ((cd.kmer & BIT63) ? cd.pos : (L - cd.pos - (uint32_t) k)); }
                        if (lane == 0) { pa[slot] = (PosT) C; reinterpret_cast<unsigned long long *>(a.kstats[6])[id] = seqHash; }
                    }
                }
            }
            if (!LONG && !FALLBACK_NOSTATS(a)) {
                unsigned char *cl = reinterpret_cast<unsigned char *>(a.kstats[4]);
                if (cl) {
                    unsigned short *ln = reinterpret_cast<unsigned short *>(cl + (size_t) id * KMC_LINE);
                    if ((uint32_t) lane < KMC_POS) ln[4 + lane] = ((uint32_t) lane < C) ? (unsigned short) cand[lane].pos : (unsigned short) 0xFFFFu;
                    if (lane == 0) *reinterpret_cast<unsigned long long *>(ln) = seqHash;
                    if (lane == 63) ln[KMC_FLAGS] = (unsigned short) KMC_CLEAN;
                }
            }
            stRes += L; stRec += 1 + C;
            __syncthreads();
            continue;
        }
        uint32_t P = 1; while (P < C) P <<= 1;
        if (P > cap) P = cap;
        for (uint32_t i = C + lane; i < P; i += 64) { Cand cd; cd.kmer = ~0ULL; cd.pos = 0xFFFFFFFFu; cd.score = 0xFFFFFFFFu; cand[i] = cd; }
        __syncthreads();
        bool sortedNeeded = true;
        if (sortedNeeded && C > 1) waveBitonicSortCands(cand, P, NUCL);
        if (a.ignoreMulti) {
            bool rep = false;
            for (uint32_t i = 1 + lane; i < C; i += 64) {
                const uint64_t x = NUCL ? (cand[i].kmer | BIT63) : cand[i].kmer, y = NUCL ? (cand[i - 1].kmer | BIT63) : cand[i - 1].kmer;
                rep |= (x == y);
            }
            if (__ballot(rep)) {
                for (uint32_t i = lane; i < C; i += 64) cand[i].score |= 0x80000000u;
                __syncthreads();
                if (lane == 0) {
                    uint32_t i = 0;
                    while (i < C) {
                        const uint64_t km = NUCL ? (cand[i].kmer | BIT63) : cand[i].kmer;
                        if (i + 1 < C && (NUCL ? (cand[i + 1].kmer | BIT63) : cand[i + 1].kmer) == km) {
                            do { i++; if (i >= C) break; } while ((NUCL ? (cand[i].kmer | BIT63) : cand[i].kmer) == km);
                            if (i >= C) break;
                        }
                        cand[i].score &= 0x7FFFFFFFu;
                        i++;
                    }
                }
                __syncthreads();
            }
        }
        uint32_t binCarry = 0, selCarry = 0;
        PosT *posCache = nullptr;
        if constexpr (NUCL) { if (!FALLBACK_NOSTATS(a)) posCache = reinterpret_cast<PosT *>(a.kstats[5]); }
        for (uint32_t c0 = 0; c0 < C; c0 += 64) {
            const uint32_t i = c0 + lane;
            Cand cd; cd.kmer = 0; cd.pos = 0; cd.score = 0x80000000u;
            if (i < C) cd = cand[i];
            const bool v = (i < C) && !(cd.score & 0x80000000u);
            const uint32_t sc = cd.score & 0xFFFFu;
            const bool isBin = v && sc == sStar;
            const unsigned long long mb = __ballot(isBin);
            const uint32_t binRank = binCarry + (uint32_t) __popcll(mb & ((1ULL << lane) - 1ULL));
            const bool selectable = v && (sc < sStar || (isBin && (tooMuch == 0 || (int) binRank < tooMuch)));
            const unsigned long long ms = __ballot(selectable);
            const uint32_t selRank = selCarry + (uint32_t) __popcll(ms & ((1ULL << lane) - 1ULL));
            if (selectable && (size_t) selRank < considered) {
                R r; r.kmer = cd.kmer; r.id = id; r.len = (decltype(r.len)) L; r.pos = (decltype(r.pos)) cd.pos;
                if constexpr (LONG) r.pad = 0;
                arr[slot + 1 + selRank] = r;
                if (selRank < 64u) sKmcPos[selRank] = (unsigned short) cd.pos;
                if constexpr (NUCL) { if (posCache) posCache[slot + 1 + selRank] = (PosT) ((cd.kmer & BIT63) ? cd.pos : (L - cd.pos - (uint32_t) k)); }
            }
            binCarry += (uint32_t) __popcll(mb); selCarry += (uint32_t) __popcll(ms);
        }
        const uint32_t numSel = (uint32_t) min((size_t) selCarry, considered);
        if constexpr (NUCL) { if (posCache && lane == 0) { posCache[slot] = (PosT) numSel; reinterpret_cast<unsigned long long *>(a.kstats[6])[id] = seqHash; } }
        if (!LONG && !FALLBACK_NOSTATS(a)) {
            unsigned char *cl = reinterpret_cast<unsigned char *>(a.kstats[4]);
            if (cl) {
                __syncthreads();
                unsigned short *ln = reinterpret_cast<unsigned short *>(cl + (size_t) id * KMC_LINE);
                if ((uint32_t) lane < KMC_POS) ln[4 + lane] = ((uint32_t) lane < numSel) ? sKmcPos[lane] : (unsigned short) 0xFFFFu;
                if (lane == 0) *reinterpret_cast<unsigned long long *>(ln) = seqHash;
                if (lane == 63) ln[KMC_FLAGS] = 0;
            }
        }
        if (lane == 0) {
            R r; r.kmer = xxh64U64(seqHash, a.seed); r.id = id; r.len = (decltype(r.len)) L; r.pos = 0;
            if constexpr (LONG) r.pad = 0;
            arr[slot] = r;
        }
        for (uint32_t i = 1 + numSel + lane; i < bound; i += 64) {
            R r; memset(&r, 0xFF, sizeof(R));
            arr[slot + i] = r;
        }
        stRes += L; stRec += 1 + numSel;
        __syncthreads();
    }
    if (lane == 0 && a.kstats) { atomicAdd(&a.kstats[2], stRes); atomicAdd(&a.kstats[3], stRec); }
}

constexpr uint32_t SHORT_MAXL = 128;
struct ShortArgs {
    SeqView s; const uint64_t *slotOff; void *arr; const unsigned char *map;
    int k, xCode, kps, ignoreMulti; float scale; uint64_t seed;
    uint64_t base, top, inv; int tz;
    uint32_t topLo, topHi, baseH;
    uint32_t *waveList, *waveCount;
    uint32_t *longList, *longCount; uint32_t longWindows;
    uint32_t *hugeList, *hugeCount; uint32_t hugeWindows;
    unsigned long long *kstats;
    uint32_t idLo, idHi; uint64_t slotBias;
    const unsigned char *changed; uint32_t *cachedList, *cachedCount;
};

template <bool LONG>
__global__ __launch_bounds__(64) void extractShortKernel(ShortArgs a) {
    __shared__ unsigned char sMap[256];
    __shared__ __attribute__((aligned(16))) unsigned short sSet[64 * 64];
    typedef Rec<LONG> R;
    R *arr = reinterpret_cast<R *>(a.arr);
    const int lane = threadIdx.x;
    for (int i = lane; i < 256; i += 64) sMap[i] = a.map[i];
    __syncthreads();
    unsigned short *mySet = sSet + lane * 64;
    const int k = a.k;
    unsigned long long stRes = 0, stRec = 0;
    for (uint32_t b0 = a.idLo + blockIdx.x * 64; b0 < a.idHi; b0 += gridDim.x * 64) {
        const uint32_t id = b0 + lane;
        const bool active = id < a.idHi;
        bool toWave = false, lenWave = false;
        if (active) {
            const uint32_t L = a.s.len[id];
            const uint32_t nWin = (L >= (uint32_t) k) ? (L - k + 1) : 0;
            const size_t consideredRaw = (size_t) ((float) (a.kps - 1) + (a.scale * (float) L));
            if (L > SHORT_MAXL || (size_t) nWin > consideredRaw) toWave = lenWave = true;
            else {
                const char *base = a.s.data + a.s.off[id];
                const uint64_t slot = a.slotOff[id] - a.slotBias;
                const uint32_t bound = (uint32_t) (a.slotOff[id + 1] - a.slotOff[id]);
                if (a.ignoreMulti) { uint4 z = make_uint4(0, 0, 0, 0); uint4 *q = reinterpret_cast<uint4 *>(mySet); for (int i = 0; i < 8; i++) q[i] = z; }
                uint64_t idx = 0, seqHash = 0, fifoLo = 0, fifoHi = 0;
                uint64_t pw = 1;
                int lastX = -1;
                uint32_t nOut = 0;
                uint32_t word = 0;
                R pend0, pend1, pend2;
                for (uint32_t i = 0; i < L; i++) {
                    if ((i & 3) == 0) __builtin_memcpy(&word, base + i, 4);
                    const unsigned char c = sMap[(word >> (8 * (i & 3))) & 0xFF];
                    seqHash = seqHash * 31 + c;
                    if (c == (unsigned char) a.xCode) lastX = (int) i;
                    if (i < (uint32_t) k) {
                        idx += (uint64_t) c * pw; pw *= a.base;
                        if (i < 8) fifoLo |= (uint64_t) c << (8 * i); else fifoHi |= (uint64_t) c << (8 * (i - 8));
                    } else {
                        const uint64_t cOut = fifoLo & 0xFF;
                        idx = (((idx - cOut) >> a.tz) * a.inv) + (uint64_t) c * a.top;
                        fifoLo = (fifoLo >> 8) | (fifoHi << 56); fifoHi >>= 8;
                        if (k - 1 < 8) fifoLo |= (uint64_t) c << (8 * (k - 1)); else fifoHi |= (uint64_t) c << (8 * (k - 1 - 8));
                    }
                    if (i + 1 >= (uint32_t) k) {
                        const uint32_t p = i + 1 - k;
                        if (lastX < (int) p) {
                            const uint32_t score = (uint32_t) ((idx * 0x9E3779B97F4A7C15ULL) >> 48);
                            if (a.ignoreMulti) {
                                const unsigned short tag = (unsigned short) (score + 1);
                                if (tag == 0 || nOut >= 48) toWave = true;
                                else {
                                    uint32_t sl = (score * 40503u >> 7) & 63;
                                    for (;;) { const unsigned short v = mySet[sl]; if (v == tag) { toWave = true; break; } if (v == 0) { mySet[sl] = tag; break; } sl = (sl + 1) & 63; }
                                }
                            }
                            R r; r.kmer = idx; r.id = id; r.len = (decltype(r.len)) L; r.pos = (decltype(r.pos)) p;
                            if constexpr (LONG) r.pad = 0;
                            switch (nOut & 3u) { case 0: pend0 = r; break; case 1: pend1 = r; break; case 2: pend2 = r; break;
                                default: { R *d = arr + slot + 1 + (nOut - 3u); d[0] = pend0; d[1] = pend1; d[2] = pend2; d[3] = r; } }
                            nOut++;
                        }
                    }
                }
                if (!toWave) {
                    { R *d = arr + slot + 1 + (nOut & ~3u); const uint32_t rem = nOut & 3u; if (rem > 0) d[0] = pend0; if (rem > 1) d[1] = pend1; if (rem > 2) d[2] = pend2; }
                    R r; r.kmer = xxh64U64(seqHash, a.seed); r.id = id; r.len = (decltype(r.len)) L; r.pos = 0;
                    if constexpr (LONG) r.pad = 0;
                    arr[slot] = r;
                    R sen; memset(&sen, 0xFF, sizeof(R));
                    for (uint32_t i = 1 + nOut; i < bound; i++) arr[slot + i] = sen;
                    stRes += L; stRec += 1 + nOut;
                }
            }
        }
        const bool isCached = lenWave && a.cachedList && a.changed[id] == 0;
        if (isCached) toWave = false;
        const uint32_t nw = (toWave && active && a.s.len[id] >= (uint32_t) k) ? a.s.len[id] - (uint32_t) k + 1 : 0u;
        const bool isHuge = toWave && a.hugeList && nw > a.hugeWindows;
        const bool isLong = toWave && !isHuge && a.longList && nw > a.longWindows;
        auto append = [&](bool mine, uint32_t *list, uint32_t *count) {
            const unsigned long long m = __ballot(mine);
            if (!m) return;
            uint32_t basePos = 0;
            if (lane == 0) basePos = atomicAdd(count, (uint32_t) __popcll(m));
            basePos = __shfl(basePos, 0, 64);
            if (mine) list[basePos + (uint32_t) __popcll(m & ((1ULL << lane) - 1ULL))] = id;
        };
        append(toWave && !isLong && !isHuge, a.waveList, a.waveCount);
        if (a.longList) append(isLong, a.longList, a.longCount);
        if (a.hugeList) append(isHuge, a.hugeList, a.hugeCount);
        if (a.cachedList) append(isCached, a.cachedList, a.cachedCount);
    }
    stRes = waveReduceSumU64(stRes); stRec = waveReduceSumU64(stRec);
    if (lane == 0 && a.kstats) { atomicAdd(&a.kstats[0], stRes); atomicAdd(&a.kstats[1], stRec); }
}

__global__ __launch_bounds__(256) void classifyWindowsKernel(const uint32_t *__restrict__ len, uint32_t idLo, uint32_t idHi, uint32_t k, uint32_t longWindows, uint32_t hugeWindows,
                                                             uint32_t *__restrict__ waveList, uint32_t *__restrict__ waveCount, uint32_t *__restrict__ longList, uint32_t *__restrict__ longCount,
                                                             uint32_t *__restrict__ hugeList, uint32_t *__restrict__ hugeCount,
                                                             const uint32_t *__restrict__ origin, uint32_t *__restrict__ cachedList, uint32_t *__restrict__ cachedCount) {
    __shared__ uint32_t sCnt[4], sBase[4];
    constexpr int PER = 8;
    for (uint64_t b0 = (uint64_t) idLo + (uint64_t) blockIdx.x * (256 * PER); b0 < idHi; b0 += (uint64_t) gridDim.x * (256 * PER)) {
        if (threadIdx.x < 4) sCnt[threadIdx.x] = 0;
        __syncthreads();
        int cls[PER]; uint32_t rank[PER];
#pragma unroll
        for (int j = 0; j < PER; j++) {
            const uint64_t id = b0 + (uint64_t) j * 256 + threadIdx.x;
            cls[j] = -1; rank[j] = 0;
            if (id < idHi) {
                const uint32_t L = len[id], nw = L >= k ? L - k + 1 : 0u;
                cls[j] = nw > hugeWindows ? 2 : (nw > longWindows ? 1 : 0);
                if (origin && origin[id] != 0xFFFFFFFFu) cls[j] = 3;
                rank[j] = atomicAdd(&sCnt[cls[j]], 1u);
            }
        }
        __syncthreads();
        if (threadIdx.x < 4) sBase[threadIdx.x] = sCnt[threadIdx.x] ? atomicAdd(threadIdx.x == 0 ? waveCount : (threadIdx.x == 1 ? longCount : (threadIdx.x == 2 ? hugeCount : cachedCount)), sCnt[threadIdx.x]) : 0u;
        __syncthreads();
#pragma unroll
        for (int j = 0; j < PER; j++)
            if (cls[j] >= 0) (cls[j] == 0 ? waveList : (cls[j] == 1 ? longList : (cls[j] == 2 ? hugeList : cachedList)))[sBase[cls[j]] + rank[j]] = (uint32_t) (b0 + (uint64_t) j * 256 + threadIdx.x);
        __syncthreads();
    }
}

__device__ __forceinline__ uint32_t mulU24(uint32_t a, uint32_t b) { uint32_t r; asm("v_mul_u32_u24_e32 %0, %1, %2" : "=v"(r) : "v"(a), "v"(b)); return r; }
__device__ __forceinline__ uint32_t waveMaxU32(uint32_t v) {
#pragma unroll
    for (int o = 32; o > 0; o >>= 1) v = max(v, (uint32_t) __shfl_xor((int) v, o, 64));
    return v;
}
template <bool LONG, int K, bool MUL24, bool STAGE = false>
__global__ __launch_bounds__(64) void extractShortFastKernel(ShortArgs a) {
    static_assert(!(STAGE && LONG), "the staging rows hold 16-byte records");
    constexpr int H = K / 2;
    static_assert(K <= 16 && 16 - K + H + 3 <= 15, "the digits that leave the halves are read from the 16-byte FIFO before this iteration's codes enter it");
    __shared__ unsigned char sMap[256];
    __shared__ __attribute__((aligned(16))) unsigned short sSet[64 * 64];
    typedef Rec<LONG> R;
    __shared__ __attribute__((aligned(16))) R sStage[STAGE ? 8 * 64 : 1];
    __shared__ unsigned long long sDst[STAGE ? 64 : 1];
    __shared__ uint32_t sCnt[STAGE ? 64 : 1];
    R *arr = reinterpret_cast<R *>(a.arr);
    const int lane = threadIdx.x;
    for (int i = lane; i < 256; i += 64) sMap[i] = a.map[i];
    __syncthreads();
    unsigned short *mySet = sSet + lane * 64;
    const uint32_t inv32 = (uint32_t) a.inv, tz = (uint32_t) a.tz, topLo = a.topLo, topHi = a.topHi, xCode = (uint32_t) a.xCode;
    const uint32_t baseH = a.baseH;
    const bool multi = a.ignoreMulti != 0;
    auto digitMul = [&](uint32_t d, uint32_t pw) -> uint32_t { return MUL24 ? __umul24(d, pw) : d * pw; };
    unsigned long long stRes = 0, stRec = 0;
    struct Ahead { uint32_t L; uint64_t off, slot, slot1; };
    auto loadAhead = [&](uint64_t idw) { Ahead m; m.L = 0; m.off = 0; m.slot = 0; m.slot1 = 0; if (idw < (uint64_t) a.idHi) { m.L = a.s.len[idw]; m.off = a.s.off[idw]; m.slot = a.slotOff[idw]; m.slot1 = a.slotOff[idw + 1]; } return m; };
    auto isShort = [&](uint32_t Lx) { const uint32_t nw = (Lx >= (uint32_t) K) ? (Lx - K + 1) : 0; const size_t cr = (size_t) ((float) (a.kps - 1) + (a.scale * (float) Lx)); return !(Lx > SHORT_MAXL || (size_t) nw > cr || (multi && nw > 48)); };
    auto firstBytes = [&](const Ahead &m, uint64_t idw) { uint4 v = make_uint4(0, 0, 0, 0); if (idw < (uint64_t) a.idHi && m.L && isShort(m.L)) __builtin_memcpy(&v, a.s.data + m.off, 16); return v; };
    constexpr bool AHEAD = !STAGE;
    const uint64_t strideIds = (uint64_t) gridDim.x * 64;
    uint64_t bw = (uint64_t) a.idLo + (uint64_t) blockIdx.x * 64;
    Ahead mCur = {0, 0, 0, 0}, mNext = {0, 0, 0, 0};
    uint4 bytesCur = make_uint4(0, 0, 0, 0);
    if (AHEAD) { mCur = loadAhead(bw + lane); mNext = loadAhead(bw + strideIds + lane); bytesCur = firstBytes(mCur, bw + lane); }
    for (uint32_t b0 = a.idLo + blockIdx.x * 64; b0 < a.idHi; b0 += gridDim.x * 64, bw += strideIds) {
        const uint32_t id = b0 + lane;
        const bool active = id < a.idHi;
        Ahead cur; uint4 curBytes;
        if (AHEAD) {
            cur = mCur; curBytes = bytesCur;
            mCur = mNext; bytesCur = firstBytes(mCur, bw + strideIds + lane);
            mNext = loadAhead(bw + 2 * strideIds + lane);
        } else { cur = loadAhead(bw + lane); curBytes = firstBytes(cur, bw + lane); }
        bool toWave = false, lenWave = false;
        uint32_t L = 0;
        if (active) {
            L = cur.L;
            const uint32_t nWin = (L >= (uint32_t) K) ? (L - K + 1) : 0;
            const size_t consideredRaw = (size_t) ((float) (a.kps - 1) + (a.scale * (float) L));
            if (L > SHORT_MAXL || (size_t) nWin > consideredRaw || (multi && nWin > 48)) toWave = lenWave = true;
        }
        const bool work = active && !toWave;
        const uint32_t Lmax = (uint32_t) __builtin_amdgcn_readfirstlane((int) waveMaxU32(work ? L : 0u));
        if (Lmax) {
            const char *base = a.s.data;
            uint64_t slot = 0; uint32_t bound = 0;
            if (work) {
                base += cur.off;
                slot = cur.slot - a.slotBias; bound = (uint32_t) (cur.slot1 - cur.slot);
                if (multi) { uint4 z = make_uint4(0, 0, 0, 0); uint4 *q = reinterpret_cast<uint4 *>(mySet); for (int i = 0; i < 8; i++) q[i] = z; }
            }
            const uint32_t Lw = work ? L : 0u;
            uint32_t lo = 0, hi = 0, f0 = 0, f1 = 0, f2 = 0, f3 = 0, nOut = 0;
            uint32_t nFlushed = 0;
            auto flush = [&]() {
                const uint32_t cnt = (work && !toWave) ? nOut - nFlushed : 0u;
                if (__ballot(cnt != 0u)) {
                    sDst[STAGE ? lane : 0] = slot + 1 + nFlushed; sCnt[STAGE ? lane : 0] = cnt;
                    __syncthreads();
#pragma unroll
                    for (int r8 = 0; r8 < 8; r8++) {
                        const int sl = r8 * 8 + (lane >> 3), j = lane & 7;
                        if ((uint32_t) j < sCnt[STAGE ? sl : 0]) arr[sDst[STAGE ? sl : 0] + (uint32_t) j] = sStage[STAGE ? (j * 64 + ((sl + 8 * j) & 63)) : 0];
                    }
                    __syncthreads();
                }
                nFlushed = nOut;
            };
            uint64_t seqHash = 0;
            int lastX = -1;
            uint4 bufNext = Lw ? curBytes : make_uint4(0, 0, 0, 0);
            for (uint32_t i0 = 0; i0 < Lmax; i0 += 16) {
                const uint4 buf = bufNext;
                bufNext = make_uint4(0, 0, 0, 0);
                if (i0 + 16 < Lw) __builtin_memcpy(&bufNext, base + i0 + 16, 16);
#pragma unroll
              for (int step = 0; step < 4; step++) {
                const uint32_t i = i0 + 4u * (uint32_t) step;
                if (i >= Lmax) break;
                const uint32_t word = step == 0 ? buf.x : (step == 1 ? buf.y : (step == 2 ? buf.z : buf.w));
                const uint32_t cw = (uint32_t) sMap[word & 0xFFu] | ((uint32_t) sMap[(word >> 8) & 0xFFu] << 8) |
                                    ((uint32_t) sMap[(word >> 16) & 0xFFu] << 16) | ((uint32_t) sMap[word >> 24] << 24);
                const uint32_t f[4] = {f0, f1, f2, f3};
                uint32_t part = 0, mult = 1;
#pragma unroll
                for (int j = 0; j < 4; j++) {
                    const bool in = i + (uint32_t) j < Lw;
                    const uint32_t c = (cw >> (8 * j)) & 0xFFu;
                    part = in ? __umul24(part, 31u) + c : part;
                    mult = in ? __umul24(mult, 31u) : mult;
                }
                seqHash = seqHash * (uint64_t) mult + (uint64_t) part;
#pragma unroll
                for (int j = 0; j < 4; j++) {
                    const uint32_t ii = i + (uint32_t) j;
                    const bool in = ii < Lw;
                    const uint32_t c = (cw >> (8 * j)) & 0xFFu;
                    lastX = (in && c == xCode) ? (int) ii : lastX;
                    constexpr int B0 = 16 - K, BH = 16 - K + H;
                    const uint32_t d0 = (f[(B0 + j) >> 2] >> (8 * ((B0 + j) & 3))) & 0xFFu;
                    const uint32_t dh = (f[(BH + j) >> 2] >> (8 * ((BH + j) & 3))) & 0xFFu;
                    lo = ((lo - d0) >> tz) * inv32 + digitMul(dh, topLo);
                    hi = ((hi - dh) >> tz) * inv32 + digitMul(c, topHi);
                    const int p = (int) ii + 1 - K;
                    if (in && !toWave && p >= 0 && lastX < p) {
                        if (multi) {
                            const uint32_t t = mulU24(lo, 0x9E3779u) ^ mulU24(hi, 0x85EBCBu) ^ (lo >> 9) ^ (hi >> 7);
                            const unsigned short tag = (unsigned short) max((t >> 8) & 0xFFFFu, 1u);
                            uint32_t sl = (t >> 3) & 63u;
                            unsigned short v = mySet[sl];
                            while (v != 0 && v != tag) { sl = (sl + 1) & 63u; v = mySet[sl]; }
                            if (v == tag) toWave = true; else mySet[sl] = tag;
                        }
                        R r; r.kmer = (uint64_t) lo + (uint64_t) hi * (uint64_t) baseH; r.id = id; r.len = (decltype(r.len)) L; r.pos = (decltype(r.pos)) p;
                        if constexpr (LONG) r.pad = 0;
                        if constexpr (STAGE) { const uint32_t pi = nOut - nFlushed; sStage[pi * 64u + (((uint32_t) lane + 8u * pi) & 63u)] = r; }
                        else arr[slot + 1 + nOut] = r;
                        nOut++;
                    }
                }
                f0 = f1; f1 = f2; f2 = f3; f3 = cw;
                if constexpr (STAGE) { if (step & 1) flush(); }
              }
            }
            if constexpr (STAGE) flush();
            if (work && !toWave) {
                R r; r.kmer = xxh64U64(seqHash, a.seed); r.id = id; r.len = (decltype(r.len)) L; r.pos = 0;
                if constexpr (LONG) r.pad = 0;
                arr[slot] = r;
                R sen; memset(&sen, 0xFF, sizeof(R));
                for (uint32_t i = 1 + nOut; i < bound; i++) arr[slot + i] = sen;
                stRes += L; stRec += 1 + nOut;
            }
        }
        const bool isCached = lenWave && a.cachedList && a.changed[id] == 0;
        if (isCached) toWave = false;
        const uint32_t nw = (toWave && active && L >= (uint32_t) K) ? L - (uint32_t) K + 1 : 0u;
        const bool isHuge = toWave && a.hugeList && nw > a.hugeWindows;
        const bool isLong = toWave && !isHuge && a.longList && nw > a.longWindows;
        auto append = [&](bool mine, uint32_t *list, uint32_t *count) {
            const unsigned long long m = __ballot(mine);
            if (!m) return;
            uint32_t basePos = 0;
            if (lane == 0) basePos = atomicAdd(count, (uint32_t) __popcll(m));
            basePos = __shfl(basePos, 0, 64);
            if (mine) list[basePos + (uint32_t) __popcll(m & ((1ULL << lane) - 1ULL))] = id;
        };
        append(toWave && !isLong && !isHuge, a.waveList, a.waveCount);
        if (a.longList) append(isLong, a.longList, a.longCount);
        if (a.hugeList) append(isHuge, a.hugeList, a.hugeCount);
        if (a.cachedList) append(isCached, a.cachedList, a.cachedCount);
    }
    stRes = waveReduceSumU64(stRes); stRec = waveReduceSumU64(stRec);
    if (lane == 0 && a.kstats) { atomicAdd(&a.kstats[0], stRes); atomicAdd(&a.kstats[1], stRec); }
}

struct CachedArgs {
    SeqView s; const uint64_t *slotOff; void *arr; const unsigned char *map; const unsigned char *lines;
    const uint32_t *list, *count; int k, xCode; uint32_t base, base7; uint64_t slotBias, seed; unsigned long long *kstats;
};
__global__ __launch_bounds__(64) void extractCachedKernel(CachedArgs a) {
    __shared__ unsigned char sMap[256];
    typedef Rec<false> R;
    R *arr = reinterpret_cast<R *>(a.arr);
    const int lane = threadIdx.x;
    for (int i = lane; i < 256; i += 64) sMap[i] = a.map[i];
    __syncthreads();
    const uint32_t nWork = *a.count;
    unsigned long long stRes = 0, stRec = 0;
    struct Meta { uint32_t id, L, pos; uint64_t off, slot, slot1; unsigned long long idh; };
    auto loadMeta = [&](uint32_t id) {
        Meta m; m.id = id; m.L = a.s.len[id]; m.off = a.s.off[id]; m.slot = a.slotOff[id] - a.slotBias; m.slot1 = a.slotOff[id + 1] - a.slotBias;
        const unsigned short *ln = reinterpret_cast<const unsigned short *>(a.lines + (size_t) id * KMC_LINE);
        m.pos = ((uint32_t) lane < KMC_POS) ? (uint32_t) ln[4 + lane] : 0xFFFFu;
        m.idh = *reinterpret_cast<const unsigned long long *>(ln);
        return m;
    };
    Meta nxt; nxt.id = 0; nxt.L = 0; nxt.pos = 0xFFFFu; nxt.off = 0; nxt.slot = 0; nxt.slot1 = 0; nxt.idh = 0;
    uint32_t id2 = 0;
    if (blockIdx.x < nWork) nxt = loadMeta(a.list[blockIdx.x]);
    if (blockIdx.x + gridDim.x < nWork) id2 = a.list[blockIdx.x + gridDim.x];
    for (uint32_t w = blockIdx.x; w < nWork; w += gridDim.x) {
        const Meta cur = nxt;
        if (w + gridDim.x < nWork) nxt = loadMeta(id2);
        if (w + 2 * gridDim.x < nWork) id2 = a.list[w + 2 * gridDim.x];
        const char *base = a.s.data + cur.off;
        const uint32_t bound = (uint32_t) (cur.slot1 - cur.slot);
        const bool have = cur.pos != 0xFFFFu;
        const uint32_t n = (uint32_t) __popcll(__ballot(have));
        if (have) {
            uint64_t r0, r1; __builtin_memcpy(&r0, base + cur.pos, 8); __builtin_memcpy(&r1, base + cur.pos + 8, 8);
            uint64_t w0 = 0, w1 = 0;
#pragma unroll
            for (int b = 0; b < 8; b++) { w0 |= (uint64_t) sMap[(r0 >> (8 * b)) & 0xFF] << (8 * b); w1 |= (uint64_t) sMap[(r1 >> (8 * b)) & 0xFF] << (8 * b); }
            uint64_t kmer; (void) kmerIndexCore(w0, w1, a.k, (unsigned) a.xCode, a.base, a.base7, kmer);
            R r; r.kmer = kmer; r.id = cur.id; r.len = (uint16_t) cur.L; r.pos = (int16_t) cur.pos;
            arr[cur.slot + 1 + (uint32_t) lane] = r;
        }
        if (lane == 63) { R r; r.kmer = xxh64U64(cur.idh, a.seed); r.id = cur.id; r.len = (uint16_t) cur.L; r.pos = 0; arr[cur.slot] = r; }
        for (uint32_t i = 1 + n + (uint32_t) lane; i < bound; i += 64) { R r; memset(&r, 0xFF, sizeof(R)); arr[cur.slot + i] = r; }
        stRes += cur.L; stRec += 1 + n;
    }
    if (lane == 0 && a.kstats) { atomicAdd(&a.kstats[2], stRes); atomicAdd(&a.kstats[3], stRec); }
}

struct RowArgs {
    SeqView s; const uint64_t *slotOff; void *arr; const unsigned char *map;
    const uint32_t *list, *count;
    uint32_t *fallList, *fallCount;
    int k, xCode, kps, ignoreMulti; uint64_t seed; uint32_t base, base7; uint64_t slotBias;
    unsigned long long *kstats;
};
constexpr uint64_t rowPowU64(uint64_t b, unsigned e) { uint64_t r = 1; while (e) { if (e & 1u) r *= b; b *= b; e >>= 1; } return r; }
constexpr uint64_t rowInv31() { uint64_t x = 31; for (int i = 0; i < 6; i++) x *= 2ull - 31ull * x; return x; }
static_assert(rowInv31() * 31ull == 1ull, "inverse of 31 modulo 2^64");
__device__ __forceinline__ uint32_t rowExclusiveScan16(uint32_t v) {
    uint32_t x = v;
    x += (uint32_t) __builtin_amdgcn_update_dpp(0, (int) x, 0x111, 0xF, 0xF, true);
    x += (uint32_t) __builtin_amdgcn_update_dpp(0, (int) x, 0x112, 0xF, 0xF, true);
    x += (uint32_t) __builtin_amdgcn_update_dpp(0, (int) x, 0x114, 0xF, 0xF, true);
    x += (uint32_t) __builtin_amdgcn_update_dpp(0, (int) x, 0x118, 0xF, 0xF, true);
    return x - v;
}
__device__ __forceinline__ unsigned long long rowSum16U64(unsigned long long v) {
    v += dppMov64<0xB1>(v); v += dppMov64<0x4E>(v); v += dppMov64<0x141>(v); v += dppMov64<0x140>(v);
    return v;
}
__global__ __launch_bounds__(256) void binWaveListKernel(const uint32_t *__restrict__ list, const uint32_t *__restrict__ count, const uint32_t *__restrict__ len, uint32_t k,
                                                         uint32_t w0, uint32_t w1, uint32_t w2, uint32_t *__restrict__ out, uint32_t outStride, uint32_t *__restrict__ outCount) {
    __shared__ uint32_t sCnt[4], sBase[4];
    const uint32_t n = *count;
    constexpr int PER = 8;
    for (uint64_t b0 = (uint64_t) blockIdx.x * (256 * PER); b0 < n; b0 += (uint64_t) gridDim.x * (256 * PER)) {
        if (threadIdx.x < 4) sCnt[threadIdx.x] = 0;
        __syncthreads();
        int cls[PER]; uint32_t rank[PER], ids[PER];
#pragma unroll
        for (int j = 0; j < PER; j++) {
            const uint64_t i = b0 + (uint64_t) j * 256 + threadIdx.x;
            cls[j] = -1; rank[j] = 0; ids[j] = 0;
            if (i < n) {
                ids[j] = list[i];
                const uint32_t L = len[ids[j]], nw = L >= k ? L - k + 1 : 0u;
                cls[j] = nw <= w0 ? 0 : (nw <= w1 ? 1 : (nw <= w2 ? 2 : 3));
                rank[j] = atomicAdd(&sCnt[cls[j]], 1u);
            }
        }
        __syncthreads();
        if (threadIdx.x < 4) sBase[threadIdx.x] = sCnt[threadIdx.x] ? atomicAdd(&outCount[threadIdx.x], sCnt[threadIdx.x]) : 0u;
        __syncthreads();
#pragma unroll
        for (int j = 0; j < PER; j++) if (cls[j] >= 0) out[(size_t) cls[j] * outStride + sBase[cls[j]] + rank[j]] = ids[j];
        __syncthreads();
    }
}

template <int REGS>
__global__ __launch_bounds__(64) __attribute__((amdgpu_waves_per_eu(4))) void extractRowKernel(RowArgs a) {
    constexpr uint32_t MAXWIN = 16u * REGS, MAXL = MAXWIN + 13u;
    constexpr uint32_t ROWB = (MAXL + 31u + 15u) & ~15u;
    constexpr bool TWO = MAXL > 256u;
    constexpr uint32_t NPOW = MAXL + 17u;
    __shared__ unsigned char sMap[256];
    __shared__ __attribute__((aligned(16))) unsigned char sCode[4][ROWB];
    __shared__ unsigned long long sPow[NPOW];
    __shared__ unsigned short sSel[4][64];
    __shared__ __attribute__((aligned(16))) uint32_t sSet[4][128];
    typedef Rec<false> R;
    R *arr = reinterpret_cast<R *>(a.arr);
    const int lane = threadIdx.x, row = lane >> 4, sub = lane & 15;
    const int k = a.k;
    if (blockIdx.x * 4u >= *a.count) return;
    for (int i = lane; i < 256; i += 64) sMap[i] = a.map[i];
    {
        constexpr uint64_t inv31 = rowInv31(), c0 = rowPowU64(inv31, 15), p64 = rowPowU64(31ull, 64);
        uint64_t m = c0;
#pragma unroll
        for (int b = 0; b < 6; b++) if ((lane >> b) & 1) m *= rowPowU64(31ull, 1u << b);
        for (uint32_t x = lane; x < NPOW; x += 64) { sPow[x] = m; m *= p64; }
    }
    __syncthreads();
    const uint32_t nWork = *a.count;
    const uint32_t stride = gridDim.x * 4u;
    const uint32_t xC = (uint32_t) a.xCode;
    const uint32_t considerRaw = (uint32_t) (a.kps - 1);
    unsigned long long stRes = 0, stRec = 0;
    struct Meta { uint32_t id, L; uint64_t off, slot, slot1; };
    auto loadMeta = [&](uint32_t w) {
        Meta m; m.id = 0xFFFFFFFFu; m.L = 0; m.off = 0; m.slot = 0; m.slot1 = 0;
        if (w < nWork) { m.id = a.list[w]; m.L = a.s.len[m.id]; m.off = a.s.off[m.id]; m.slot = a.slotOff[m.id] - a.slotBias; m.slot1 = a.slotOff[m.id + 1] - a.slotBias; }
        return m;
    };
    auto loadRaw = [&](const Meta &m, uint32_t at) { uint4 v = make_uint4(0, 0, 0, 0); if (at < m.L) __builtin_memcpy(&v, a.s.data + m.off + at, 16); return v; };
    uint32_t w = blockIdx.x * 4u + (uint32_t) row;
    auto loadId = [&](uint32_t ww) { return ww < nWork ? a.list[ww] : 0xFFFFFFFFu; };
    auto metaOf = [&](uint32_t id) {
        Meta m; m.id = id; m.L = 0; m.off = 0; m.slot = 0; m.slot1 = 0;
        if (id != 0xFFFFFFFFu) { m.L = a.s.len[id]; m.off = a.s.off[id]; m.slot = a.slotOff[id] - a.slotBias; m.slot1 = a.slotOff[id + 1] - a.slotBias; }
        return m;
    };
    Meta mNext = loadMeta(w); uint32_t id2 = loadId(w + stride);
    uint4 rawN0 = loadRaw(mNext, (uint32_t) sub * 16u);
    for (uint32_t w0 = blockIdx.x * 4u; w0 < nWork; w0 += stride, w += stride) {
        const Meta cur = mNext; const uint4 raw0 = rawN0;
        uint4 raw1 = make_uint4(0, 0, 0, 0);
        if (TWO) raw1 = loadRaw(cur, 256u + (uint32_t) sub * 16u);
        mNext = metaOf(id2);
        rawN0 = loadRaw(mNext, (uint32_t) sub * 16u);
        id2 = loadId(w + 2u * stride);
        const bool active = cur.id != 0xFFFFFFFFu;
        const uint32_t L = cur.L, id = cur.id;
        const uint32_t nWin = (L >= (uint32_t) k) ? L - (uint32_t) k + 1u : 0u;
        const bool tooLong = active && nWin > MAXWIN;
        const uint32_t nWinU = (uint32_t) __builtin_amdgcn_readfirstlane((int) waveMaxU32((active && !tooLong) ? nWin : 0u));
        unsigned long long hAcc = 0;
        auto stageChunk = [&](const uint4 &raw, uint32_t c) {
            const uint32_t r[4] = {raw.x, raw.y, raw.z, raw.w};
            uint32_t cw[4];
#pragma unroll
            for (int d = 0; d < 4; d++)
                cw[d] = (uint32_t) sMap[r[d] & 0xFFu] | ((uint32_t) sMap[(r[d] >> 8) & 0xFFu] << 8) | ((uint32_t) sMap[(r[d] >> 16) & 0xFFu] << 16) | ((uint32_t) sMap[r[d] >> 24] << 24);
            if (16u * c < ROWB) *reinterpret_cast<uint4 *>(&sCode[row][16u * c]) = make_uint4(cw[0], cw[1], cw[2], cw[3]);
            const int m = (int) L - (int) (16u * c);
            if (m > 0 && !tooLong) {
                uint32_t q[4];
#pragma unroll
                for (int d = 0; d < 4; d++) {
                    const int nb = m - 4 * d;
                    const uint32_t z = nb >= 4 ? cw[d] : (nb <= 0 ? 0u : (cw[d] & ((1u << (8 * nb)) - 1u)));
                    q[d] = __umul24(__umul24(__umul24(z & 0xFFu, 31u) + ((z >> 8) & 0xFFu), 31u) + ((z >> 16) & 0xFFu), 31u) + (z >> 24);
                }
                constexpr unsigned long long K4 = 923521ull;
                const unsigned long long H = (((unsigned long long) q[0] * K4 + q[1]) * K4 + q[2]) * K4 + q[3];
                hAcc += H * sPow[(uint32_t) ((int) L - 16 * (int) (c + 1) + 15)];
            }
        };
        stageChunk(raw0, (uint32_t) sub);
        if (TWO) stageChunk(raw1, 16u + (uint32_t) sub);
        if (active && !tooLong) for (uint32_t i = (uint32_t) sub; i < 31u; i += 16u) sCode[row][L + i] = (unsigned char) xC;
        for (uint32_t i = (uint32_t) sub * 4u; i < 128u; i += 64u) *reinterpret_cast<uint4 *>(&sSet[row][i]) = make_uint4(0, 0, 0, 0);
        __syncthreads();
        const unsigned long long seqHash = rowSum16U64(hAcc);
        uint32_t sc[REGS];
        uint32_t nLane = 0;
#pragma unroll
        for (int j = 0; j < REGS; j++) {
            sc[j] = 0xFFFFFFFFu;
            if ((uint32_t) j * 16u < nWinU) {
                const uint32_t p = (uint32_t) j * 16u + (uint32_t) sub;
                uint64_t kmer;
                const bool v = kmerIndexFastAligned(sCode[row], p, k, xC, a.base, a.base7, kmer);
                const uint32_t h = xxh64Score16(kmer, a.seed);
                const bool use = v && p < nWin && !tooLong;
                sc[j] = use ? h : 0xFFFFFFFFu; nLane += use ? 1u : 0u;
            }
            __builtin_amdgcn_sched_barrier(0);
        }
        const uint32_t n = (uint32_t) rowSum16((int) nLane);
        const uint32_t considered = min(considerRaw, n);
        uint32_t t = 0;
#pragma unroll 1
        for (int bit = 15; bit >= 0; bit--) {
            const uint32_t tr = t | (1u << bit);
            uint32_t c = 0;
#pragma unroll
            for (int j = 0; j < REGS; j++) if ((uint32_t) j * 16u < nWinU) c += (sc[j] < tr) ? 1u : 0u;
            if ((uint32_t) rowSum16((int) c) < considered) t = tr;
        }
        if (n <= considered) t = 0xFFFFu;
        uint32_t selMask = 0;
#pragma unroll
        for (int j = 0; j < REGS; j++) if ((uint32_t) j * 16u < nWinU) selMask |= (sc[j] <= t) ? (1u << j) : 0u;
        const uint32_t cLane = (uint32_t) __popc(selMask);
        const uint32_t C = (uint32_t) rowSum16((int) cLane);
        bool ok = active && !tooLong && C == considered;
        {
            uint32_t at = rowExclusiveScan16(cLane);
            if (ok) {
#pragma unroll
                for (int j = 0; j < REGS; j++) if ((selMask >> j) & 1u) { sSel[row][at] = (unsigned short) ((uint32_t) j * 16u + (uint32_t) sub); at++; }
            }
        }
        __syncthreads();
        const uint64_t slot = cur.slot;
        const uint32_t bound = (uint32_t) (cur.slot1 - cur.slot);
        bool rep = false;
#pragma unroll
        for (int i = 0; i < 4; i++) {
            const uint32_t r = (uint32_t) sub + 16u * (uint32_t) i;
            if (ok && r < C) {
                const uint32_t p = sSel[row][r];
                uint64_t kmer; (void) kmerIndexFastAligned(sCode[row], p, k, xC, a.base, a.base7, kmer);
                if (a.ignoreMulti) {
                    const uint64_t hx = kmer * 0x9E3779B97F4A7C15ULL;
                    const uint32_t tag = (uint32_t) (hx >> 32) | 1u;
                    uint32_t sl = (uint32_t) (hx >> 20) & 127u;
                    for (;;) {
                        const uint32_t prev = atomicCAS(&sSet[row][sl], 0u, tag);
                        if (prev == 0u) break;
                        if (prev == tag) { rep = true; break; }
                        sl = (sl + 1u) & 127u;
                    }
                }
                R rec; rec.kmer = kmer; rec.id = id; rec.len = (uint16_t) L; rec.pos = (int16_t) p;
                arr[slot + 1 + r] = rec;
            }
            __builtin_amdgcn_sched_barrier(0);
        }
        if (rowSum16(rep ? 1 : 0) != 0) ok = false;
        if (ok) {
            if (sub == 15) { R rec; rec.kmer = xxh64U64(seqHash, a.seed); rec.id = id; rec.len = (uint16_t) L; rec.pos = 0; arr[slot] = rec; }
            for (uint32_t i = 1u + C + (uint32_t) sub; i < bound; i += 16u) { R rec; memset(&rec, 0xFF, sizeof(R)); arr[slot + i] = rec; }
            unsigned char *cl = reinterpret_cast<unsigned char *>(a.kstats[4]);
            if (cl) {
                unsigned short *ln = reinterpret_cast<unsigned short *>(cl + (size_t) id * KMC_LINE);
#pragma unroll
                for (int i = 0; i < 4; i++) { const uint32_t r = (uint32_t) sub + 16u * (uint32_t) i; if (r < KMC_POS) ln[4 + r] = (r < C) ? sSel[row][r] : (unsigned short) 0xFFFFu; }
                if (sub == 0) *reinterpret_cast<unsigned long long *>(ln) = seqHash;
                if (sub == 15) ln[KMC_FLAGS] = (unsigned short) KMC_CLEAN;
            }
            if (sub == 0) { stRes += L; stRec += 1 + C; }
        }
        {
            const bool fall = active && !ok && sub == 0;
            const unsigned long long fm = __ballot(fall);
            if (fm) {
                uint32_t basePos = 0;
                if (lane == 0) basePos = atomicAdd(a.fallCount, (uint32_t) __popcll(fm));
                basePos = __shfl(basePos, 0, 64);
                if (fall) a.fallList[basePos + (uint32_t) __popcll(fm & ((1ULL << lane) - 1ULL))] = id;
            }
        }
        __syncthreads();
    }
    stRes = waveReduceSumU64(stRes); stRec = waveReduceSumU64(stRec);
    if (lane == 0 && a.kstats) { atomicAdd(&a.kstats[2], stRes); atomicAdd(&a.kstats[3], stRec); }
}

template <bool LONG>
struct CachedPosArgs {
    SeqView s; const uint64_t *slotOff; void *arr; const unsigned char *map;
    const void *posOld; const uint64_t *slotOffOld; const unsigned long long *idHashOld; const uint32_t *origin;
    void *posNew; unsigned long long *idHashNew;
    const uint32_t *list, *count; int k; uint64_t seed; unsigned long long *kstats;
};
template <bool LONG>
__global__ __launch_bounds__(64) void extractCachedPosKernel(CachedPosArgs<LONG> a) {
    __shared__ unsigned char sMap[256];
    typedef Rec<LONG> R;
    typedef typename std::conditional<LONG, uint32_t, unsigned short>::type PosT;
    R *arr = reinterpret_cast<R *>(a.arr);
    const PosT *posOld = reinterpret_cast<const PosT *>(a.posOld);
    PosT *posNew = reinterpret_cast<PosT *>(a.posNew);
    const int lane = threadIdx.x;
// ... 73 lines not shown
```

Before: 718.7 million.

## Classify long sequences up front and overlap short/wave extraction on two streams

Moves classification of which sequences are too long for the per-thread short extractor into classifyWindowsKernel, which now runs before the short kernel. The short kernels no longer build the wave, long, huge and cached lists themselves. With the lists ready early, the wave-tier extract kernels can run on a second stream while the short-thread kernel runs on the main stream, joined by fork and join events. This is enabled by default only for large inputs (over 4M sequences). A leftover repeatList, which is expected to stay empty, is processed after the join. The change adds stream management and event sync, and the two kernel groups may contend for the same CUs.

```diff
diff --git a/plass_amd/csrc/common.hpp b/plass_amd/csrc/common.hpp
--- a/plass_amd/csrc/common.hpp
+++ b/plass_amd/csrc/common.hpp
@@ -103,6 +103,8 @@
     int device = 0;
     hipStream_t stream = nullptr;
     hipEvent_t ev[16] = {};
+    hipStream_t stream2 = nullptr;
+    hipEvent_t forkEv = nullptr, joinEv = nullptr;
     int numCU = 0;
     std::vector<uint32_t> ambKeys;
     std::vector<uint8_t> ambVals;
diff --git a/plass_amd/csrc/core.hip b/plass_amd/csrc/core.hip
--- a/plass_amd/csrc/core.hip
+++ b/plass_amd/csrc/core.hip
@@ -169,7 +169,7 @@
     const char *e = getenv(key); const int v = e ? atoi(e) : 0;
     return v > 0 ? v : dflt;
 }
-static const char *const TUNE_NAMES[] = {"AGGWAVE", "AGGWAVE_CAP", "ASMQ", "ASMQ_CAP", "ROWTIER", "KMCACHE", "FORCE_LONG", "CYC_PASSES", "CYCSKIP", "SHARD_EXTRACT",
+static const char *const TUNE_NAMES[] = {"AGGWAVE", "AGGWAVE_CAP", "ASMQ", "ASMQ_CAP", "ROWTIER", "EXTRACT_STREAMS", "KMCACHE", "FORCE_LONG", "CYC_PASSES", "CYCSKIP", "SHARD_EXTRACT",
                                          "FASTA_CHUNK_MB", "DBHEAP", "DBHEAP_GB", "LAZY_SELF", "FASTQ_CHUNK_KB"};
 static void reportUnknownTunes() {
     static const char PREFIX[] = "PLASSHIP_TUNE_";
@@ -264,6 +264,9 @@
     PH_CHECK(hipStreamCreateWithFlags(&c->stream, hipStreamNonBlocking));
     poolEnter(c->stream);
     for (auto &ev : c->ev) PH_CHECK(hipEventCreate(&ev));
+    PH_CHECK(hipStreamCreateWithFlags(&c->stream2, hipStreamNonBlocking));
+    PH_CHECK(hipEventCreateWithFlags(&c->forkEv, hipEventDisableTiming));
+    PH_CHECK(hipEventCreateWithFlags(&c->joinEv, hipEventDisableTiming));
     { std::lock_guard<std::mutex> g(g_poolMu); g_ctxCount++; }
     *out = holder.release();
     return PLASSHIP_OK;
@@ -294,7 +297,10 @@
     if (!ctx) return;
     (void) hipSetDevice(ctx->device);
     (void) plasship::streamSync(ctx->stream);
+    if (ctx->stream2) { (void) hipStreamSynchronize(ctx->stream2); (void) hipStreamDestroy(ctx->stream2); }
     for (auto &ev : ctx->ev) if (ev) (void) hipEventDestroy(ev);
+    if (ctx->forkEv) (void) hipEventDestroy(ctx->forkEv);
+    if (ctx->joinEv) (void) hipEventDestroy(ctx->joinEv);
     for (int i = 0; i < 2; i++) { if (ctx->stage[i]) (void) hipHostFree(ctx->stage[i]); if (ctx->stageEv[i]) (void) hipEventDestroy(ctx->stageEv[i]); }
     if (ctx->pinnedTable) (void) hipHostFree(ctx->pinnedTable);
     { std::unique_lock<std::mutex> lk(g_reserveMu); g_reserveCv.wait(lk, [] { return g_reserving == 0; }); }
diff --git a/plass_amd/csrc/kmermatch.hip b/plass_amd/csrc/kmermatch.hip
--- a/plass_amd/csrc/kmermatch.hip
+++ b/plass_amd/csrc/kmermatch.hip
@@ -836,20 +836,45 @@
     }
     PH_CHECK(hipMemcpyAsync(dKStats.as<unsigned long long>() + 4, cachePtrs, 24, hipMemcpyHostToDevice, st));
     PH_CHECK(hipEventRecord(ctx->ev[2], st));
-    if (!NUCL && k <= 16 && nMine) {
+    const bool threadKernel = !NUCL && k <= 16;
+    constexpr int KF = 14, HF = KF / 2;
+    uint64_t pwH = 1; for (int i = 0; i < HF; i++) pwH *= (uint64_t) (alph - 1);
+    const bool fast = k == KF && pwH * 2 < (1ull << 32);
+    DevBuf dRepList, dRepCnt, dOv2Ids, dOv2Cnt, dRowLists, dRowCounts, dRowFall, dRowFallCnt;
+    const bool rowTier = !NUCL && !LONG && fastIndex && k <= 14 && par->kmers_per_seq >= 1 && par->kmers_per_seq <= (int) KMC_POS + 1 &&
+                         par->kmers_per_seq_scale == 0.0f && (tuneInt("ROWTIER", nMine > 4000000u ? 1 : 2) & 1) == 1;
+    const uint32_t rs = N + 1;
+    if (nMine) {
+        if (dOv2Ids.alloc(((size_t) N + 1) * 4) != hipSuccess || dOv2Cnt.alloc(4) != hipSuccess || dRepCnt.alloc(4) != hipSuccess || (threadKernel && dRepList.alloc(((size_t) N + 1) * 4) != hipSuccess) ||
+            (rowTier && (dRowLists.alloc((size_t) 4 * rs * 4) != hipSuccess || dRowCounts.alloc(16) != hipSuccess || dRowFall.alloc((size_t) rs * 4) != hipSuccess || dRowFallCnt.alloc(4) != hipSuccess))) {
+            setError("kmermatch: out of device memory"); return PLASSHIP_ERR_DEVICE;
+        }
+        PH_CHECK(hipMemsetAsync(dOv2Cnt.p, 0, 4, st));
+        PH_CHECK(hipMemsetAsync(dRepCnt.p, 0, 4, st));
+        if (rowTier) { PH_CHECK(hipMemsetAsync(dRowCounts.p, 0, 16, st)); PH_CHECK(hipMemsetAsync(dRowFallCnt.p, 0, 4, st)); }
+        ShortClass sc; memset(&sc, 0, sizeof(sc));
+        if (threadKernel) { sc.on = 1; sc.kps = par->kmers_per_seq; sc.cap48 = (fast && par->ignore_multi_kmer) ? 1 : 0; sc.scale = par->kmers_per_seq_scale; sc.changed = cacheReuse ? db->d_changed.as<unsigned char>() : nullptr; }
+        hipLaunchKernelGGL(classifyWindowsKernel, dim3(std::min<uint32_t>((nMine + 2047) / 2048, (uint32_t) ctx->numCU * 8)), dim3(256), 0, st, (const uint32_t *) db->d_len.as<uint32_t>(), sLo, sHi, (uint32_t) k,
+                           TIER0_WINDOWS, 64u * 16u, dWaveList.as<uint32_t>(), dWaveCount.as<uint32_t>(), dLongList.as<uint32_t>(), dLongCount.as<uint32_t>(), dOvIds.as<uint32_t>(), dOvCnt.as<uint32_t>(),
+                           (NUCL && posReuse) ? (const uint32_t *) db->d_origin.as<uint32_t>() : (const uint32_t *) nullptr, dCachedList.as<uint32_t>(), dCachedCount.as<uint32_t>(), sc);
+        ea.waveList = dWaveList.as<uint32_t>(); ea.waveCount = dWaveCount.as<uint32_t>();
+    }
+    const bool twoStreams = threadKernel && nMine && !cm && tuneInt("EXTRACT_STREAMS", nMine > 4000000u ? 2 : 1) == 2;
+    hipStream_t sw = twoStreams ? ctx->stream2 : st;
+    struct ForkGuard { hipStream_t s = nullptr; ~ForkGuard() { if (s) (void) hipStreamSynchronize(s); } } forkGuard;
+    if (twoStreams) {
+        PH_CHECK(hipEventRecord(ctx->forkEv, st));
+        PH_CHECK(hipStreamWaitEvent(sw, ctx->forkEv, 0));
+        forkGuard.s = sw;
+        PH_CHECK(hipEventRecord(ctx->ev[4], sw));
+    }
+    if (threadKernel && nMine) {
         ShortArgs sa; memset(&sa, 0, sizeof(sa));
         sa.s = ea.s; sa.slotOff = ea.slotOff; sa.arr = ea.arr; sa.map = ea.map; sa.k = k; sa.xCode = ea.xCode; sa.kps = ea.kps; sa.ignoreMulti = ea.ignoreMulti;
         sa.scale = ea.scale; sa.seed = ea.seed; sa.base = (uint64_t) (alph - 1); sa.top = ea.powers[k - 1];
         { uint64_t b = sa.base; int tz = 0; while ((b & 1) == 0) { b >>= 1; tz++; } uint64_t inv = b; for (int i = 0; i < 6; i++) inv *= 2 - b * inv; sa.tz = tz; sa.inv = inv; }
-        sa.waveList = dWaveList.as<uint32_t>(); sa.waveCount = dWaveCount.as<uint32_t>(); sa.kstats = dKStats.as<unsigned long long>();
-        sa.longList = dLongList.as<uint32_t>(); sa.longCount = dLongCount.as<uint32_t>(); sa.longWindows = TIER0_WINDOWS;
-        sa.hugeList = dOvIds.as<uint32_t>(); sa.hugeCount = dOvCnt.as<uint32_t>(); sa.hugeWindows = 64 * 16;
+        sa.repeatList = dRepList.as<uint32_t>(); sa.repeatCount = dRepCnt.as<uint32_t>(); sa.kstats = dKStats.as<unsigned long long>();
         sa.idLo = sLo; sa.idHi = sHi; sa.slotBias = slotBias;
-        if (cacheReuse) { sa.changed = db->d_changed.as<unsigned char>(); sa.cachedList = dCachedList.as<uint32_t>(); sa.cachedCount = dCachedCount.as<uint32_t>(); }
-        constexpr int KF = 14, HF = KF / 2;
-        bool fast = k == KF;
-        uint64_t pwH = 1; for (int i = 0; i < HF; i++) pwH *= sa.base;
-        if (pwH * 2 >= (1ull << 32)) fast = false;
         sa.topLo = (uint32_t) (pwH / sa.base); sa.topHi = (uint32_t) ea.powers[KF - HF - 1]; sa.baseH = (uint32_t) pwH;
         const dim3 shortGrid(std::min<uint32_t>((nMine + 63) / 64, (uint32_t) ctx->numCU * (nMine > 20000000u ? 288u : 18u)));
         const bool allWork = (int64_t) db->maxEntryLen - 2 - k + 1 <= (int64_t) par->kmers_per_seq - 1;
@@ -861,7 +886,6 @@
         else if (fast && sa.base < (1u << 8) && sa.topLo < (1u << 24) && sa.topHi < (1u << 24)) hipLaunchKernelGGL((extractShortFastKernel<LONG, KF, true>), shortGrid, dim3(64), padLds, st, sa);
         else if (fast) hipLaunchKernelGGL((extractShortFastKernel<LONG, KF, false>), shortGrid, dim3(64), 0, st, sa);
         else hipLaunchKernelGGL((extractShortKernel<LONG>), shortGrid, dim3(64), 0, st, sa);
-        ea.waveList = dWaveList.as<uint32_t>(); ea.waveCount = dWaveCount.as<uint32_t>();
         if (cacheReuse) {
             CachedArgs ca; memset(&ca, 0, sizeof(ca));
             ca.s = ea.s; ca.slotOff = ea.slotOff; ca.arr = ea.arr; ca.map = ea.map; ca.lines = kc.lines.as<unsigned char>();
@@ -871,10 +895,6 @@
         }
     }
     else if (nMine) {
-        hipLaunchKernelGGL(classifyWindowsKernel, dim3(std::min<uint32_t>((nMine + 2047) / 2048, (uint32_t) ctx->numCU * 8)), dim3(256), 0, st, (const uint32_t *) db->d_len.as<uint32_t>(), sLo, sHi, (uint32_t) k,
-                           TIER0_WINDOWS, 64u * 16u, dWaveList.as<uint32_t>(), dWaveCount.as<uint32_t>(), dLongList.as<uint32_t>(), dLongCount.as<uint32_t>(), dOvIds.as<uint32_t>(), dOvCnt.as<uint32_t>(),
-                           posReuse ? (const uint32_t *) db->d_origin.as<uint32_t>() : (const uint32_t *) nullptr, dCachedList.as<uint32_t>(), dCachedCount.as<uint32_t>());
-        ea.waveList = dWaveList.as<uint32_t>(); ea.waveCount = dWaveCount.as<uint32_t>();
         if constexpr (NUCL) {
             if (posReuse) {
                 CachedPosArgs<LONG> ca; memset(&ca, 0, sizeof(ca));
@@ -886,26 +906,14 @@
         }
     }
     PH_CHECK(hipEventRecord(ctx->ev[3], st));
-    PH_CHECK(hipEventRecord(ctx->ev[4], st));
+    if (!twoStreams) PH_CHECK(hipEventRecord(ctx->ev[4], st));
     const int waveBlocksPerCU = nMine > 5000000u ? 192 : 32;
-    DevBuf dOv2Ids, dOv2Cnt;
     DevBuf *lastIds = &dOvIds, *lastCnt = &dOvCnt;
     if (nMine) {
-        if (dOv2Ids.alloc(((size_t) N + 1) * 4) != hipSuccess || dOv2Cnt.alloc(4) != hipSuccess) { setError("kmermatch: out of device memory"); return PLASSHIP_ERR_DEVICE; }
-        PH_CHECK(hipMemsetAsync(dOv2Cnt.p, 0, 4, st));
         const uint32_t wide = std::min<uint32_t>(nMine, (uint32_t) ctx->numCU * (uint32_t) waveBlocksPerCU);
         ExtractArgs e0 = ea;
-        DevBuf dRowLists, dRowCounts, dRowFall, dRowFallCnt;
-        const bool rowTier = !NUCL && !LONG && fastIndex && k <= 14 && par->kmers_per_seq >= 1 && par->kmers_per_seq <= (int) KMC_POS + 1 &&
-                             par->kmers_per_seq_scale == 0.0f && (tuneInt("ROWTIER", nMine > 4000000u ? 1 : 2) & 1) == 1;
         if (rowTier) {
-            const uint32_t rs = N + 1;
-            if (dRowLists.alloc((size_t) 4 * rs * 4) != hipSuccess || dRowCounts.alloc(16) != hipSuccess || dRowFall.alloc((size_t) rs * 4) != hipSuccess || dRowFallCnt.alloc(4) != hipSuccess) {
-                setError("kmermatch: out of device memory"); return PLASSHIP_ERR_DEVICE;
-            }
-            PH_CHECK(hipMemsetAsync(dRowCounts.p, 0, 16, st));
-            PH_CHECK(hipMemsetAsync(dRowFallCnt.p, 0, 4, st));
-            hipLaunchKernelGGL(binWaveListKernel, dim3(std::min<uint32_t>((nMine + 2047) / 2048, (uint32_t) ctx->numCU * 8)), dim3(256), 0, st, (const uint32_t *) dWaveList.as<uint32_t>(), (const uint32_t *) dWaveCount.as<uint32_t>(),
+            hipLaunchKernelGGL(binWaveListKernel, dim3(std::min<uint32_t>((nMine + 2047) / 2048, (uint32_t) ctx->numCU * 8)), dim3(256), 0, sw, (const uint32_t *) dWaveList.as<uint32_t>(), (const uint32_t *) dWaveCount.as<uint32_t>(),
                                (const uint32_t *) db->d_len.as<uint32_t>(), (uint32_t) k, 96u, 128u, 192u, dRowLists.as<uint32_t>(), rs, dRowCounts.as<uint32_t>());
             RowArgs ra; memset(&ra, 0, sizeof(ra));
             ra.s = ea.s; ra.slotOff = ea.slotOff; ra.arr = ea.arr; ra.map = ea.map; ra.fallList = dRowFall.as<uint32_t>(); ra.fallCount = dRowFallCnt.as<uint32_t>();
@@ -914,25 +922,34 @@
             const dim3 rowGrid(std::min<uint32_t>((nMine + 3) / 4, (uint32_t) ctx->numCU * 32u));
             for (int b = 0; b < 4; b++) {
                 ra.list = dRowLists.as<uint32_t>() + (size_t) b * rs; ra.count = dRowCounts.as<uint32_t>() + b;
-                if (b == 0) hipLaunchKernelGGL((extractRowKernel<6>), rowGrid, dim3(64), 0, st, ra);
-                else if (b == 1) hipLaunchKernelGGL((extractRowKernel<8>), rowGrid, dim3(64), 0, st, ra);
-                else if (b == 2) hipLaunchKernelGGL((extractRowKernel<12>), rowGrid, dim3(64), 0, st, ra);
-                else hipLaunchKernelGGL((extractRowKernel<16>), rowGrid, dim3(64), 0, st, ra);
+                if (b == 0) hipLaunchKernelGGL((extractRowKernel<6>), rowGrid, dim3(64), 0, sw, ra);
+                else if (b == 1) hipLaunchKernelGGL((extractRowKernel<8>), rowGrid, dim3(64), 0, sw, ra);
+                else if (b == 2) hipLaunchKernelGGL((extractRowKernel<12>), rowGrid, dim3(64), 0, sw, ra);
+                else hipLaunchKernelGGL((extractRowKernel<16>), rowGrid, dim3(64), 0, sw, ra);
             }
             e0.waveList = dRowFall.as<uint32_t>(); e0.waveCount = dRowFallCnt.as<uint32_t>();
         }
-        hipLaunchKernelGGL((extractKernel<NUCL, LONG, CAP, false, 4, 256>), dim3(wide), dim3(64), 0, st, e0);
+        hipLaunchKernelGGL((extractKernel<NUCL, LONG, CAP, false, 4, 256>), dim3(wide), dim3(64), 0, sw, e0);
         ExtractArgs e1 = ea; e1.waveList = dLongList.as<uint32_t>(); e1.waveCount = dLongCount.as<uint32_t>();
-        hipLaunchKernelGGL((extractKernel<NUCL, LONG, CAP, false, 16, 992>), dim3(wide), dim3(64), 0, st, e1);
+        hipLaunchKernelGGL((extractKernel<NUCL, LONG, CAP, false, 16, 992>), dim3(wide), dim3(64), 0, sw, e1);
         ExtractArgs e2 = ea; e2.waveList = dOvIds.as<uint32_t>(); e2.waveCount = dOvCnt.as<uint32_t>();
         e2.overflowIds = dOv2Ids.as<uint32_t>(); e2.overflowCount = dOv2Cnt.as<uint32_t>();
         constexpr int CAP48 = NUCL ? 512 : 128;
-        if constexpr (NUCL) hipLaunchKernelGGL((extractKernel<NUCL, LONG, CAP48, false, 48, 992, 2>), dim3(std::min<uint32_t>(nMine, (uint32_t) ctx->numCU * 8u)), dim3(64), 0, st, e2);
-        else hipLaunchKernelGGL((extractKernel<NUCL, LONG, CAP2, false, 48, 992>), dim3(std::min<uint32_t>(nMine, (uint32_t) ctx->numCU * 16u)), dim3(64), 0, st, e2);
-        PH_CHECK(hipMemsetAsync(dOvCnt.p, 0, 4, st));
+        if constexpr (NUCL) hipLaunchKernelGGL((extractKernel<NUCL, LONG, CAP48, false, 48, 992, 2>), dim3(std::min<uint32_t>(nMine, (uint32_t) ctx->numCU * 8u)), dim3(64), 0, sw, e2);
+        else hipLaunchKernelGGL((extractKernel<NUCL, LONG, CAP2, false, 48, 992>), dim3(std::min<uint32_t>(nMine, (uint32_t) ctx->numCU * 16u)), dim3(64), 0, sw, e2);
+        PH_CHECK(hipMemsetAsync(dOvCnt.p, 0, 4, sw));
         ExtractArgs e3 = ea; e3.waveList = dOv2Ids.as<uint32_t>(); e3.waveCount = dOv2Cnt.as<uint32_t>();
         e3.overflowIds = dOvIds.as<uint32_t>(); e3.overflowCount = dOvCnt.as<uint32_t>();
-        hipLaunchKernelGGL((extractKernel<NUCL, LONG, CAP2, false, 0, 8160>), dim3(std::min<uint32_t>(nMine, (uint32_t) ctx->numCU * (NUCL ? 2u : 5u))), dim3(64), 0, st, e3);
+        hipLaunchKernelGGL((extractKernel<NUCL, LONG, CAP2, false, 0, 8160>), dim3(std::min<uint32_t>(nMine, (uint32_t) ctx->numCU * (NUCL ? 2u : 5u))), dim3(64), 0, sw, e3);
+        if (twoStreams) {
+            PH_CHECK(hipEventRecord(ctx->joinEv, sw));
+            PH_CHECK(hipStreamWaitEvent(st, ctx->joinEv, 0));
+            forkGuard.s = nullptr;
+        }
+        if (threadKernel) {
+            ExtractArgs er = ea; er.waveList = dRepList.as<uint32_t>(); er.waveCount = dRepCnt.as<uint32_t>();
+            hipLaunchKernelGGL((extractKernel<NUCL, LONG, CAP, false, 4, 256>), dim3(wide), dim3(64), 0, st, er);
+        }
     }
     DevBuf &dLastIds = *lastIds, &dLastCnt = *lastCnt;
     PH_CHECK(hipEventRecord(ctx->ev[5], st));
@@ -983,6 +1000,7 @@
             stats->n_kmer_records = lo.Nk; stats->n_grouped = lo.Nm; stats->n_candidates = NcL; stats->record_bytes = LONG ? 20 : 16;
             float ms = 0, ms2 = 0; (void) hipEventElapsedTime(&ms, ctx->ev[2], ctx->ev[3]); (void) hipEventElapsedTime(&ms2, ctx->ev[4], ctx->ev[5]);
             stats->ms_extract_short_kernel = ms; stats->ms_extract_wave_kernel = ms2; stats->ms_extract_kernel = ms + ms2;
+            if (twoStreams) (void) hipEventElapsedTime(&stats->ms_extract_kernel, ctx->ev[2], ctx->ev[5]);
             stats->ms_part_scatter = lo.msPart; stats->n_part_scatter = lo.nPart;
             unsigned long long ks[4] = {0, 0, 0, 0}; uint32_t nCachedSeqs = 0;
             if (cacheReuse || posReuse) PH_CHECK(hipMemcpyAsync(&nCachedSeqs, dCachedCount.p, 4, hipMemcpyDeviceToHost, st));
diff --git a/plass_amd/csrc/kmermatch_extract.hpp b/plass_amd/csrc/kmermatch_extract.hpp
--- a/plass_amd/csrc/kmermatch_extract.hpp
+++ b/plass_amd/csrc/kmermatch_extract.hpp
@@ -613,13 +613,15 @@
     int k, xCode, kps, ignoreMulti; float scale; uint64_t seed;
     uint64_t base, top, inv; int tz;
     uint32_t topLo, topHi, baseH;
-    uint32_t *waveList, *waveCount;
-    uint32_t *longList, *longCount; uint32_t longWindows;
-    uint32_t *hugeList, *hugeCount; uint32_t hugeWindows;
+    uint32_t *repeatList, *repeatCount;
     unsigned long long *kstats;
     uint32_t idLo, idHi; uint64_t slotBias;
-    const unsigned char *changed; uint32_t *cachedList, *cachedCount;
 };
+__device__ __forceinline__ bool tooLongForThread(uint32_t L, uint32_t k, int kps, float scale, bool cap48) {
+    const uint32_t nWin = (L >= k) ? (L - k + 1) : 0;
+    const size_t consideredRaw = (size_t) ((float) (kps - 1) + (scale * (float) L));
+    return L > SHORT_MAXL || (size_t) nWin > consideredRaw || (cap48 && nWin > 48);
+}
 
 template <bool LONG>
 __global__ __launch_bounds__(64) void extractShortKernel(ShortArgs a) {
@@ -636,13 +638,10 @@
     for (uint32_t b0 = a.idLo + blockIdx.x * 64; b0 < a.idHi; b0 += gridDim.x * 64) {
         const uint32_t id = b0 + lane;
         const bool active = id < a.idHi;
-        bool toWave = false, lenWave = false;
+        bool toWave = false;
         if (active) {
             const uint32_t L = a.s.len[id];
-            const uint32_t nWin = (L >= (uint32_t) k) ? (L - k + 1) : 0;
-            const size_t consideredRaw = (size_t) ((float) (a.kps - 1) + (a.scale * (float) L));
-            if (L > SHORT_MAXL || (size_t) nWin > consideredRaw) toWave = lenWave = true;
-            else {
+            if (!tooLongForThread(L, (uint32_t) k, a.kps, a.scale, false)) {
                 const char *base = a.s.data + a.s.off[id];
                 const uint64_t slot = a.slotOff[id] - a.slotBias;
                 const uint32_t bound = (uint32_t) (a.slotOff[id + 1] - a.slotOff[id]);
@@ -698,11 +697,6 @@
                 }
             }
         }
-        const bool isCached = lenWave && a.cachedList && a.changed[id] == 0;
-        if (isCached) toWave = false;
-        const uint32_t nw = (toWave && active && a.s.len[id] >= (uint32_t) k) ? a.s.len[id] - (uint32_t) k + 1 : 0u;
-        const bool isHuge = toWave && a.hugeList && nw > a.hugeWindows;
-        const bool isLong = toWave && !isHuge && a.longList && nw > a.longWindows;
         auto append = [&](bool mine, uint32_t *list, uint32_t *count) {
             const unsigned long long m = __ballot(mine);
             if (!m) return;
@@ -711,19 +705,17 @@
             basePos = __shfl(basePos, 0, 64);
             if (mine) list[basePos + (uint32_t) __popcll(m & ((1ULL << lane) - 1ULL))] = id;
         };
-        append(toWave && !isLong && !isHuge, a.waveList, a.waveCount);
-        if (a.longList) append(isLong, a.longList, a.longCount);
-        if (a.hugeList) append(isHuge, a.hugeList, a.hugeCount);
-        if (a.cachedList) append(isCached, a.cachedList, a.cachedCount);
+        append(toWave, a.repeatList, a.repeatCount);
     }
     stRes = waveReduceSumU64(stRes); stRec = waveReduceSumU64(stRec);
     if (lane == 0 && a.kstats) { atomicAdd(&a.kstats[0], stRes); atomicAdd(&a.kstats[1], stRec); }
 }
 
+struct ShortClass { int on, kps, cap48; float scale; const unsigned char *changed; };
 __global__ __launch_bounds__(256) void classifyWindowsKernel(const uint32_t *__restrict__ len, uint32_t idLo, uint32_t idHi, uint32_t k, uint32_t longWindows, uint32_t hugeWindows,
                                                              uint32_t *__restrict__ waveList, uint32_t *__restrict__ waveCount, uint32_t *__restrict__ longList, uint32_t *__restrict__ longCount,
                                                              uint32_t *__restrict__ hugeList, uint32_t *__restrict__ hugeCount,
-                                                             const uint32_t *__restrict__ origin, uint32_t *__restrict__ cachedList, uint32_t *__restrict__ cachedCount) {
+                                                             const uint32_t *__restrict__ origin, uint32_t *__restrict__ cachedList, uint32_t *__restrict__ cachedCount, ShortClass sc) {
     __shared__ uint32_t sCnt[4], sBase[4];
     constexpr int PER = 8;
     for (uint64_t b0 = (uint64_t) idLo + (uint64_t) blockIdx.x * (256 * PER); b0 < idHi; b0 += (uint64_t) gridDim.x * (256 * PER)) {
@@ -738,7 +730,8 @@
                 const uint32_t L = len[id], nw = L >= k ? L - k + 1 : 0u;
                 cls[j] = nw > hugeWindows ? 2 : (nw > longWindows ? 1 : 0);
                 if (origin && origin[id] != 0xFFFFFFFFu) cls[j] = 3;
-                rank[j] = atomicAdd(&sCnt[cls[j]], 1u);
+                if (sc.on) { if (!tooLongForThread(L, k, sc.kps, sc.scale, sc.cap48 != 0)) cls[j] = -1; else if (sc.changed && sc.changed[id] == 0) cls[j] = 3; }
+                if (cls[j] >= 0) rank[j] = atomicAdd(&sCnt[cls[j]], 1u);
             }
         }
         __syncthreads();
@@ -780,7 +773,7 @@
     unsigned long long stRes = 0, stRec = 0;
     struct Ahead { uint32_t L; uint64_t off, slot, slot1; };
     auto loadAhead = [&](uint64_t idw) { Ahead m; m.L = 0; m.off = 0; m.slot = 0; m.slot1 = 0; if (idw < (uint64_t) a.idHi) { m.L = a.s.len[idw]; m.off = a.s.off[idw]; m.slot = a.slotOff[idw]; m.slot1 = a.slotOff[idw + 1]; } return m; };
-    auto isShort = [&](uint32_t Lx) { const uint32_t nw = (Lx >= (uint32_t) K) ? (Lx - K + 1) : 0; const size_t cr = (size_t) ((float) (a.kps - 1) + (a.scale * (float) Lx)); return !(Lx > SHORT_MAXL || (size_t) nw > cr || (multi && nw > 48)); };
+    auto isShort = [&](uint32_t Lx) { return !tooLongForThread(Lx, (uint32_t) K, a.kps, a.scale, multi); };
     auto firstBytes = [&](const Ahead &m, uint64_t idw) { uint4 v = make_uint4(0, 0, 0, 0); if (idw < (uint64_t) a.idHi && m.L && isShort(m.L)) __builtin_memcpy(&v, a.s.data + m.off, 16); return v; };
     constexpr bool AHEAD = !STAGE;
     const uint64_t strideIds = (uint64_t) gridDim.x * 64;
@@ -797,15 +790,10 @@
             mCur = mNext; bytesCur = firstBytes(mCur, bw + strideIds + lane);
             mNext = loadAhead(bw + 2 * strideIds + lane);
         } else { cur = loadAhead(bw + lane); curBytes = firstBytes(cur, bw + lane); }
-        bool toWave = false, lenWave = false;
+        bool toWave = false;
         uint32_t L = 0;
-        if (active) {
-            L = cur.L;
-            const uint32_t nWin = (L >= (uint32_t) K) ? (L - K + 1) : 0;
-            const size_t consideredRaw = (size_t) ((float) (a.kps - 1) + (a.scale * (float) L));
-            if (L > SHORT_MAXL || (size_t) nWin > consideredRaw || (multi && nWin > 48)) toWave = lenWave = true;
-        }
-        const bool work = active && !toWave;
+        if (active) L = cur.L;
+        const bool work = active && !tooLongForThread(L, (uint32_t) K, a.kps, a.scale, multi);
         const uint32_t Lmax = (uint32_t) __builtin_amdgcn_readfirstlane((int) waveMaxU32(work ? L : 0u));
         if (Lmax) {
             const char *base = a.s.data;
@@ -898,11 +886,6 @@
                 stRes += L; stRec += 1 + nOut;
             }
         }
-        const bool isCached = lenWave && a.cachedList && a.changed[id] == 0;
-        if (isCached) toWave = false;
-        const uint32_t nw = (toWave && active && L >= (uint32_t) K) ? L - (uint32_t) K + 1 : 0u;
-        const bool isHuge = toWave && a.hugeList && nw > a.hugeWindows;
-        const bool isLong = toWave && !isHuge && a.longList && nw > a.longWindows;
         auto append = [&](bool mine, uint32_t *list, uint32_t *count) {
             const unsigned long long m = __ballot(mine);
             if (!m) return;
@@ -911,10 +894,7 @@
             basePos = __shfl(basePos, 0, 64);
             if (mine) list[basePos + (uint32_t) __popcll(m & ((1ULL << lane) - 1ULL))] = id;
         };
-        append(toWave && !isLong && !isHuge, a.waveList, a.waveCount);
-        if (a.longList) append(isLong, a.longList, a.longCount);
-        if (a.hugeList) append(isHuge, a.hugeList, a.hugeCount);
-        if (a.cachedList) append(isCached, a.cachedList, a.cachedCount);
+        append(toWave, a.repeatList, a.repeatCount);
     }
     stRes = waveReduceSumU64(stRes); stRec = waveReduceSumU64(stRec);
     if (lane == 0 && a.kstats) { atomicAdd(&a.kstats[0], stRes); atomicAdd(&a.kstats[1], stRec); }
```

New measurement: 704.3 million. -2.0%, worse.
